# MiniMax-AI/VTP

Hardware: AMD Instinct MI355X
Metric: images/sec/node VTP-B f16d64 256x256 train step (higher is better)
Workload: dtype bf16

## Files before the change

### vtp_amd/csrc/gemm.hip

```cpp
#include "common.h"
#include "gemm_common.h"
#include <cstdlib>

namespace vtp {


template <int BM, int BN, int WAVES_M, int WAVES_N, int STAGES, int EPI, bool TRANS, bool PIPE>
__global__ __launch_bounds__(64 * WAVES_M* WAVES_N) void gemm_nt_kernel(const GemmArgs p_in) {
  constexpr int BK = 64;
  GemmArgs p = p_in;
  if constexpr (!TRANS) {
    if (p.m_rows) p.M = min(p.M, __builtin_amdgcn_readfirstlane(*p.m_rows));
  }
  constexpr int NW = WAVES_M * WAVES_N;
  constexpr int WTM = BM / WAVES_M, WTN = BN / WAVES_N;
  constexpr int TM = WTM / 32, TN = WTN / 32;
  constexpr int A_BYTES = BM * BK * 2, B_BYTES = BN * BK * 2, STAGE_BYTES = A_BYTES + B_BYTES;
  constexpr int PA = BM / 8 / NW, PB = BN / 8 / NW;
  constexpr int P = PA + PB;
  static_assert(PA >= 1 && PB >= 1 && TM >= 1 && TN >= 1, "bad tile config");
  static_assert(STAGES == 2 || STAGES == 3, "2 or 3 stages");
  extern __shared__ __attribute__((aligned(16))) char smem[];

  const int tid = threadIdx.x;
  const int lane = tid & 63;
  const int wave = __builtin_amdgcn_readfirstlane(tid >> 6);
  const int wm = wave % WAVES_M, wn = wave / WAVES_M;
  const int hi = lane >> 5;

  const int tiles_m = (p.M + BM - 1) / BM;
  const int tiles_n = (p.N + BN - 1) / BN;
  const int ntiles = tiles_m * tiles_n;
  const int G = gridDim.x;
  const int n_my = (ntiles - (int)blockIdx.x + G - 1) / G;
  auto tile_origin = [&](int i, int& m0, int& n0) {
    int wg = blockIdx.x + i * G;
    if (p.xcd_swizzle & 1) wg = xcd_chunk_start(wg, ntiles) + (wg >> 3);
    n0 = (wg % tiles_n) * BN;
    m0 = (wg / tiles_n) * BM;
  };
  const int kbeg = blockIdx.z * p.k_split;
  const int kend = min(p.K, kbeg + p.k_split);
  const int nk = (kend - kbeg + BK - 1) / BK;

  const int prow = lane >> 3;
  const int slot = lane & 7;
  const char* a_src[PA];
  const char* b_src[PB];
  int a_kc[PA], b_kc[PB];
  const char* zsrc = (const char*)g_zero_block;
  auto set_src = [&](int m0, int n0) {
    if constexpr (!TRANS) {
  #pragma unroll
      for (int i = 0; i < PA; ++i) {
        const int row = (wave * PA + i) * 8 + prow;
        const int c = slot ^ ((row >> 1) & 7);
        int m = min(m0 + row, p.M - 1);
        m = remap_row(m, p.a_grp, p.a_pre);
        a_src[i] = (const char*)(p.A + (size_t)m * p.lda + kbeg + c * 8);
        a_kc[i] = c * 8;
      }
  #pragma unroll
      for (int i = 0; i < PB; ++i) {
        const int row = (wave * PB + i) * 8 + prow;
        const int c = slot ^ ((row >> 1) & 7);
        const int n = min(n0 + row, p.N - 1);
        b_src[i] = (const char*)(p.B + (size_t)n * p.ldb + kbeg + c * 8);
        b_kc[i] = c * 8;
      }
    } else {
  #pragma unroll
      for (int i = 0; i < PA; ++i) {
        const int byte = (wave * PA + i) * 1024 + lane * 16;
        const int r = byte / (BM * 2);
        const int sp = (byte % (BM * 2)) >> 4;
        const int col = m0 + ((sp ^ (4 * (r & 3))) << 3);
        a_kc[i] = r;
        a_src[i] = col < p.M ? (const char*)(p.A + col) : nullptr;
      }
  #pragma unroll
      for (int i = 0; i < PB; ++i) {
        const int byte = (wave * PB + i) * 1024 + lane * 16;
        const int r = byte / (BN * 2);
        const int sp = (byte % (BN * 2)) >> 4;
        const int col = n0 + ((sp ^ (4 * (r & 3))) << 3);
        b_kc[i] = r;
        b_src[i] = col < p.N ? (const char*)(p.B + col) : nullptr;
      }
    }
  };

  auto stage_part = [&](int buf, int kt, int q) {
    char* abase = smem + buf * STAGE_BYTES;
    char* bbase = abase + A_BYTES;
    const int krem = kend - kbeg - kt * BK;
#pragma unroll
    for (int i = 0; i < PA; ++i) {
      if (q >= 0 && (i & 3) != q) continue;
      const char* s;
      if constexpr (!TRANS) {
        if constexpr (EPI == EPI_CONV_RELU || EPI == EPI_CONV_MASK) {
          long off = (long)kt * (BK * 2);
          if (p.conv_cin) {
            const int k0 = kt * BK, tap = k0 / p.conv_cin;
            const int ky = tap / 3, kx = tap - 3 * ky;
            off = ((long)((ky - 1) * p.conv_w2 + (kx - 1)) * p.lda + (k0 - tap * p.conv_cin)) * 2;
          }
          s = (a_kc[i] < krem) ? a_src[i] + off : zsrc;
        } else {
          s = (a_kc[i] < krem) ? a_src[i] + (size_t)kt * (BK * 2) : zsrc;
        }
      } else {
        const int t = kbeg + kt * BK + a_kc[i];
        s = (a_kc[i] < krem && a_src[i]) ? a_src[i] + (size_t)remap_row(t, p.a_grp, p.a_pre) * p.lda * 2 : zsrc;
      }
      __builtin_amdgcn_global_load_lds((const __attribute__((address_space(1))) void*)s,
                                       (__attribute__((address_space(3))) void*)(abase + (wave * PA + i) * 1024),
                                       16, 0, 0);
    }
#pragma unroll
    for (int i = 0; i < PB; ++i) {
      if (q >= 0 && ((i + PA) & 3) != q) continue;
      const char* s;
      if constexpr (!TRANS) {
        s = (b_kc[i] < krem) ? b_src[i] + (size_t)kt * (BK * 2) : zsrc;
      } else {
        const int t = kbeg + kt * BK + b_kc[i];
        s = (b_kc[i] < krem && b_src[i]) ? b_src[i] + (size_t)remap_row(t, p.b_grp, p.b_pre) * p.ldb * 2 : zsrc;
      }
      __builtin_amdgcn_global_load_lds((const __attribute__((address_space(1))) void*)s,
                                       (__attribute__((address_space(3))) void*)(bbase + (wave * PB + i) * 1024),
                                       16, 0, 0);
    }
  };
  auto stage = [&](int buf, int kt) { stage_part(buf, kt, -1); };

  f32x16 acc[TN][TM];
#pragma unroll
  for (int i = 0; i < TN; ++i)
#pragma unroll
    for (int j = 0; j < TM; ++j)
#pragma unroll
      for (int r = 0; r < 16; ++r) acc[i][j][r] = 0.f;

  const int sw = (lane >> 1) & 7;
  const int rowoff = (lane & 31) * 128;

  int s_i = 0, s_kt = 0;
  {
    int m0s, n0s;
    tile_origin(0, m0s, n0s);
    set_src(m0s, n0s);
  }
  auto advance = [&]() {
    if (++s_kt == nk) {
      s_kt = 0;
      if (++s_i < n_my) {
        int m0s, n0s;
        tile_origin(s_i, m0s, n0s);
        set_src(m0s, n0s);
      }
    }
  };
#pragma unroll
  for (int s = 0; s < STAGES - 1; ++s)
    if (s_i < n_my) {
      stage(s, s_kt);
      advance();
    }

  int buf = 0;
  int landed = 0;
  for (int ti = 0; ti < n_my; ++ti) {
  int m0, n0;
  tile_origin(ti, m0, n0);
  for (int kt = 0; kt < nk; ++kt) {
    if (landed > 0) {
      --landed;
    } else {
      const int rem = (n_my - 1 - ti) * nk + (nk - 1 - kt);
      const int later = min(STAGES - 2, rem);
      if (later >= 2) wait_vmcnt<2 * P>();
      else if (later == 1) wait_vmcnt<P>();
      else wait_vmcnt<0>();
    }
    __builtin_amdgcn_s_barrier();
    asm volatile("" ::: "memory");
    const bool prefetch = s_i < n_my;
    int nb = buf + STAGES - 1;
    if (nb >= STAGES) nb -= STAGES;
    if (!PIPE && prefetch) {
      stage(nb, s_kt);
      advance();
    }
    const char* abase = smem + buf * STAGE_BYTES;
    const char* bbase = abase + A_BYTES;

    auto load_frags = [&](int ks, bf16x8* wf, bf16x8* xf) {
      if constexpr (!TRANS) {
        const int coff = ((2 * ks + hi) ^ sw) << 4;
#pragma unroll
        for (int i = 0; i < TN; ++i)
          wf[i] = *(const bf16x8*)(bbase + (wn * WTN + i * 32) * 128 + rowoff + coff);
#pragma unroll
        for (int j = 0; j < TM; ++j)
          xf[j] = *(const bf16x8*)(abase + (wm * WTM + j * 32) * 128 + rowoff + coff);
      } else {
        const int li = lane & 15, lg = (lane >> 4) & 1;
        const int rq = li >> 2;
        const int cin = lg * 16 + (li & 3) * 4;
#pragma unroll
        for (int i = 0; i < TN; ++i) {
          const int col = wn * WTN + i * 32 + cin;
          const int soff = (((col >> 3) ^ (4 * rq)) << 4) + ((col & 7) << 1);
          const char* b0 = bbase + (ks * 16 + hi * 8 + rq) * (BN * 2) + soff;
          bf16x4 lo = __builtin_amdgcn_ds_read_tr16_b64_v4bf16((__attribute__((address_space(3))) bf16x4*)b0);
          bf16x4 hi4 = __builtin_amdgcn_ds_read_tr16_b64_v4bf16((__attribute__((address_space(3))) bf16x4*)(b0 + 4 * (BN * 2)));
          wf[i] = __builtin_shufflevector(lo, hi4, 0, 1, 2, 3, 4, 5, 6, 7);
        }
#pragma unroll
        for (int j = 0; j < TM; ++j) {
          const int col = wm * WTM + j * 32 + cin;
          const int soff = (((col >> 3) ^ (4 * rq)) << 4) + ((col & 7) << 1);
          const char* a0 = abase + (ks * 16 + hi * 8 + rq) * (BM * 2) + soff;
          bf16x4 lo = __builtin_amdgcn_ds_read_tr16_b64_v4bf16((__attribute__((address_space(3))) bf16x4*)a0);
          bf16x4 hi4 = __builtin_amdgcn_ds_read_tr16_b64_v4bf16((__attribute__((address_space(3))) bf16x4*)(a0 + 4 * (BM * 2)));
          xf[j] = __builtin_shufflevector(lo, hi4, 0, 1, 2, 3, 4, 5, 6, 7);
        }
      }
    };

    if constexpr (PIPE) {
      bf16x8 wf[2][TN], xf[2][TM];
      load_frags(0, wf[0], xf[0]);
#pragma unroll
      for (int ks = 0; ks < 4; ++ks) {
        if (ks < 3) load_frags(ks + 1, wf[(ks + 1) & 1], xf[(ks + 1) & 1]);
        if (prefetch) stage_part(nb, s_kt, ks);
#pragma unroll
        for (int i = 0; i < TN; ++i)
#pragma unroll
          for (int j = 0; j < TM; ++j)
            acc[i][j] = __builtin_amdgcn_mfma_f32_32x32x16_bf16(wf[ks & 1][i], xf[ks & 1][j], acc[i][j], 0, 0, 0);
      }
      if (prefetch) advance();
    } else {
#pragma unroll
      for (int ks = 0; ks < 4; ++ks) {
        bf16x8 wf[TN], xf[TM];
        load_frags(ks, wf, xf);
#pragma unroll
        for (int i = 0; i < TN; ++i)
#pragma unroll
          for (int j = 0; j < TM; ++j)
            acc[i][j] = __builtin_amdgcn_mfma_f32_32x32x16_bf16(wf[i], xf[j], acc[i][j], 0, 0, 0);
      }
    }
    if (++buf == STAGES) buf = 0;
  }
  if (ti + 1 < n_my) {
    wait_vmcnt<0>();
    landed = min(STAGES - 1, (n_my - 1 - ti) * nk);
  }

  {
    constexpr int REGION = STAGE_BYTES / NW;
    char* reg = nullptr;
    if (gemm_epilogue_uses_lds<EPI, TRANS, WTN, REGION>(p)) {
      const int lb = (buf == 0 ? STAGES : buf) - 1;
      __builtin_amdgcn_s_barrier();
      asm volatile("" ::: "memory");
      reg = smem + lb * STAGE_BYTES + wave * REGION;
    }
    gemm_epilogue<EPI, TRANS, WTM, WTN, REGION>(p, acc, reg, m0, n0, wm, wn, lane);
  }
#pragma unroll
  for (int i = 0; i < TN; ++i)
#pragma unroll
    for (int j = 0; j < TM; ++j)
#pragma unroll
      for (int r = 0; r < 16; ++r) acc[i][j][r] = 0.f;
  }
}

template <int BM, int BN, int WAVES_M, int WAVES_N, int STAGES, int EPI, bool TRANS, bool PIPE = false>
static int launch_cfg(const GemmArgs& a, int splits, hipStream_t s) {
  constexpr int LDS = STAGES * (BM + BN) * 64 * 2;
  static bool attr_set = false;
  auto kern = gemm_nt_kernel<BM, BN, WAVES_M, WAVES_N, STAGES, EPI, TRANS, PIPE>;
  if (!attr_set) {
    hipFuncSetAttribute((const void*)kern, hipFuncAttributeMaxDynamicSharedMemorySize, LDS);
    attr_set = true;
  }
  static int slots = 0;
  if (!slots) {
    int occ = 1, dev = 0;
    hipDeviceProp_t prop;
    (void)hipGetDevice(&dev);
    (void)hipGetDeviceProperties(&prop, dev);
    (void)hipOccupancyMaxActiveBlocksPerMultiprocessor(&occ, (const void*)kern, 64 * WAVES_M * WAVES_N, LDS);
    slots = prop.multiProcessorCount * (occ < 1 ? 1 : occ);
    slots -= slots % 8;
  }
  const int ntiles = cdiv(a.M, BM) * cdiv(a.N, BN);
  dim3 grid(splits == 1 && ntiles > slots ? slots : ntiles, 1, splits);
  hipLaunchKernelGGL(kern, grid, dim3(64 * WAVES_M * WAVES_N), LDS, s, a);
  return check_launch(TRANS ? "gemm_tn" : "gemm_nt");
}

static int g_force_cfg = -1;
static int g_xcd_swizzle = 3;
static int swz_flags() { return g_xcd_swizzle; }


int launch_gemm8p_nt(const GemmArgs& a, int epi, int splits, hipStream_t s);
int launch_gemm8p_tn(const GemmArgs& a, int epi, int splits, hipStream_t s);
bool gemm8p_fits(const GemmArgs& a, bool trans);
bool gemm8p_combine_ready(hipStream_t s);
int launch_gemm8h_nt(const GemmArgs& a, int epi, hipStream_t s);
int launch_gemm4w_nt(const GemmArgs& a, int epi, hipStream_t s);

template <int EPI, bool TRANS>
static int launch_gemm(const GemmArgs& a, int splits, int cfg, hipStream_t s) {
  if (cfg == 10) {
    if constexpr (!TRANS && (EPI == EPI_BF16 || EPI == EPI_F32 || EPI == EPI_SWIGLU || EPI == EPI_GELU)) {
      if (splits == 1 && a.N % 256 == 0 && a.K % 128 == 0 && a.a_grp == 0 && a.conv_cin == 0 && !a.timing &&
          gemm8p_fits(a, false))
        return launch_gemm4w_nt(a, EPI, s);
    }
    cfg = TRANS ? 5 : 8;
  }
  if (cfg == 9) {
    if constexpr (!TRANS && (EPI == EPI_BF16 || EPI == EPI_F32 || EPI == EPI_SWIGLU || EPI == EPI_GELU)) {
      if (splits == 1 && a.N % 256 == 0 && gemm8p_fits(a, false)) return launch_gemm8h_nt(a, EPI, s);
    }
    cfg = TRANS ? 5 : 8;
  }
  if (cfg == 8) {
    if constexpr (TRANS) {
      if (a.a_grp == 0 && a.b_grp == 0 && gemm8p_fits(a, true)) return launch_gemm8p_tn(a, EPI, splits, s);
      cfg = 5;
    } else if constexpr (EPI != EPI_CONV_RELU && EPI != EPI_CONV_MASK) {
      if (gemm8p_fits(a, false)) return launch_gemm8p_nt(a, EPI, splits, s);
      cfg = 5;
    }
  }
  if constexpr (TRANS) {
    return launch_cfg<128, 128, 4, 2, 2, EPI, true>(a, splits, s);
  } else {
    switch (cfg) {
      case 3: return launch_cfg<256, 128, 4, 2, 3, EPI, false>(a, splits, s);
      case 4:
        if constexpr (EPI == EPI_BF16) return launch_cfg<256, 128, 4, 2, 2, EPI, false>(a, splits, s);
        else return launch_cfg<256, 256, 4, 2, 2, EPI, false>(a, splits, s);
      case 5: return launch_cfg<128, 128, 4, 2, 2, EPI, false>(a, splits, s);
      case 7: return launch_cfg<128, 64, 4, 1, 3, EPI, false>(a, splits, s);
      case 21: return launch_cfg<128, 128, 4, 2, 2, EPI, false, true>(a, splits, s);
      default: return launch_cfg<128, 128, 2, 2, 2, EPI, false>(a, splits, s);
    }
  }
}

static bool use_8p_nt(int M, int N, int K, int epilogue) {
  if (N < 256 || K < 256) return false;
  const int tiles = cdiv(M, 256) * cdiv(N, 256);
  if (K < 512) return epilogue == VTP_EPI_BF16 && tiles >= 1024;
  switch (epilogue) {
    case VTP_EPI_F32: return tiles >= 128;
    case VTP_EPI_SWIGLU: return tiles >= 96;
    case VTP_EPI_BF16:
    case VTP_EPI_GELU: return tiles >= (K < 1024 ? 192 : 96);
    default: return false;
  }
}

static bool use_8h_nt(const GemmArgs& a, int epilogue) {
  if (a.N % 256 != 0 || a.N < 256 || a.K < 512) return false;
  const int t256 = cdiv(a.M, 256) * (a.N / 256), t8h = cdiv(a.M, 128) * (a.N / 256);
  if (epilogue == VTP_EPI_BF16) {
    if (a.swiglu_pre) return t256 > 256;
    if (a.rope_pos) return t256 >= 192 && t256 <= 768;
    return t256 <= 128 && t8h >= 192 && a.K <= 2304;
  }
  if (epilogue == VTP_EPI_SWIGLU) return t256 > 768 && t256 <= 1280;
  return false;
}

static bool use_8p_tn(int M, int N, int K, int splits, const GemmArgs& a) {
  if (a.a_grp || a.b_grp) return false;
  const int wgs = cdiv(M, 256) * cdiv(N, 256) * splits;
  return wgs >= 160 && wgs <= 256 && K / splits >= 1024;
}

static int combine_splits(int M, int N, int K) {
  if (N < 256 || M < 1024 || K < 4096) return 1;
  const int tiles = cdiv(M, 256) * cdiv(N, 256);
  return (tiles >= 48 && tiles <= 128) ? 2 : 1;
}

static int pick_cfg(int M, int N, int K, int epilogue, int splits) {
  if (g_force_cfg >= 0) return g_force_cfg;
  if (M < 128 || N < 128) return 0;
  if (splits > 1) return 3;
  if (use_8p_nt(M, N, K, epilogue)) return 8;
  if (cdiv(M, 256) * cdiv(N, 256) >= 384 && (N >= 2304 || K >= (epilogue == VTP_EPI_F32 ? 4096 : 2048))) return 4;
  if ((epilogue == VTP_EPI_BF16 || epilogue == VTP_EPI_F32) && K >= 512 && cdiv(M, 128) * cdiv(N, 128) < 400) return 7;
  if (K >= 4096) return 21;
  if (epilogue == VTP_EPI_SWIGLU) return 0;
  return 5;
}

static bool use_4w_nt(const GemmArgs& a, int epilogue) {
  if (epilogue != VTP_EPI_BF16 || a.rope_pos || a.swiglu_pre || a.a_grp || a.conv_cin || a.timing) return false;
  if (a.N % 256 != 0 || a.K % 128 != 0 || a.K < 2048) return false;
  return cdiv(a.M, 256) * (a.N / 256) >= 192;
}

static int pick_cfg_nt(const GemmArgs& a, int epilogue, int splits) {
  const int cfg = pick_cfg(a.M, a.N, a.K, epilogue, splits);
  static const bool use_4w = [] { const char* e = getenv("VTP_GEMM4W"); return !(e && e[0] == '0'); }();
  if (use_4w && g_force_cfg < 0 && splits == 1 && use_4w_nt(a, epilogue) && gemm8p_fits(a, false)) return 10;
  static const bool use_8h = [] { const char* e = getenv("VTP_GEMM8H"); return !(e && e[0] == '0'); }();
  if (use_8h && g_force_cfg < 0 && splits == 1 && a.a_grp == 0 && use_8h_nt(a, epilogue) && gemm8p_fits(a, false)) return 9;
  return cfg;
}

}

using namespace vtp;

template <int EPI>
static int launch_conv(const GemmArgs& a, hipStream_t s) {
  if (a.N <= 64) return launch_cfg<256, 64, 4, 2, 2, EPI, false>(a, 1, s);
  if (a.N <= 128) return launch_cfg<256, 128, 4, 2, 2, EPI, false>(a, 1, s);
  return launch_cfg<256, 256, 4, 2, 2, EPI, false>(a, 1, s);
}

extern "C" int vtp_conv3x3(const void* x, const void* w, const float* bias, void* y, const void* relu_mask, int NB, int H,
                           int W, int Cin, int Cout, int taps, int mode, void* stream) {
  VTP_REQUIRE(x && w && y, "vtp_conv3x3: null operand");
  VTP_REQUIRE(NB > 0 && H > 0 && W > 0, "vtp_conv3x3: bad shape");
  VTP_REQUIRE(taps == 9 || taps == 1, "vtp_conv3x3: taps must be 9 (3x3) or 1 (pre-unfolded rows)");
  VTP_REQUIRE(Cin % 8 == 0 && Cout % 4 == 0 && (taps == 1 || Cin % 64 == 0),
              "vtp_conv3x3: Cin must be a multiple of 64 (8 for pre-unfolded rows), Cout of 4");
  VTP_REQUIRE(mode == 0 ? bias != nullptr : true, "vtp_conv3x3: forward mode needs a bias");
  GemmArgs a{};
  a.A = (const bf16*)x; a.B = (const bf16*)w; a.C = y; a.C2 = (void*)relu_mask; a.bias = bias;
  a.M = NB * (H + 2) * (W + 2); a.N = Cout; a.K = taps * Cin;
  a.lda = Cin; a.ldb = taps * Cin; a.ldc = Cout; a.ldc2 = Cout; a.alpha = 1.f;
  a.k_split = (a.K + 63) / 64 * 64;
  a.xcd_swizzle = swz_flags();
  a.conv_cin = taps == 9 ? Cin : 0; a.conv_w2 = W + 2; a.conv_h2 = H + 2; a.conv_p = (H + 2) * (W + 2);
  hipStream_t s = (hipStream_t)stream;
  return mode == 0 ? launch_conv<EPI_CONV_RELU>(a, s) : launch_conv<EPI_CONV_MASK>(a, s);
}

extern "C" int vtp_gemm_splits(int K, int splits) {
  if (splits < 1) splits = 1;
  const int ks = ((K + splits - 1) / splits + 63) / 64 * 64;
  return (K + ks - 1) / ks;
}

extern "C" int vtp_gemm_tn_splits(int M, int N, int K) {
  const int t256 = cdiv(M, 256) * cdiv(N, 256);
  int s8 = 256 / t256;
  if (s8 > K / 1024) s8 = K / 1024;
  if (g_force_cfg < 0 && s8 >= 1) {
    const int eff = vtp_gemm_splits(K, s8);
    if (t256 * eff >= 160 && t256 * eff <= 256 && K / eff >= 1024) return eff;
  }
  const int t128 = cdiv(M, 128) * cdiv(N, 128);
  int s = 512 / t128;
  if (s > K / 512) s = K / 512;
  if (s > 16) s = 16;
  if (s < 1) s = 1;
  return vtp_gemm_splits(K, s);
}

extern "C" int vtp_set_gemm_tuning(int force_cfg, int xcd_swizzle) {
  bool known = false;
  for (int id : {-1, 0, 3, 4, 5, 7, 8, 9, 10, 21}) known |= force_cfg == id;
  VTP_REQUIRE(known, "vtp_set_gemm_tuning: force_cfg %d names no kernel configuration (-1, 0, 3, 4, 5, 7, 8, 9, 10, 21)", force_cfg);
  g_force_cfg = force_cfg;
  g_xcd_swizzle = xcd_swizzle;
  return VTP_OK;
}

extern "C" int vtp_gemm_nt_config(int M, int N, int K, int epilogue) {
  if (M <= 0 || N <= 0 || K <= 0) return -1;
  GemmArgs a{};
  a.M = M; a.N = N; a.K = K; a.lda = K; a.ldb = K;
  int cfg = pick_cfg_nt(a, epilogue, 1);
  int cs = 1;
  if (g_force_cfg < 0 && epilogue <= VTP_EPI_GELU && gemm8p_fits(a, false)) cs = combine_splits(M, N, K);
  if (cs > 1) cfg = 8;
  return cfg | (cs > 1 ? cs << 8 : 0);
}

static int gemm_nt_impl(const void* A, int lda, const void* B, int ldb, void* C, int ldc, void* C2, int ldc2,
                        const float* bias, const float* gamma, const float* resid, int M, int N, int K, int epilogue,
                        int a_grp, int a_pre, int c_grp, int c_pre, int splits, float alpha, const int* m_rows, void* stream) {
  VTP_REQUIRE(A && B && C, "vtp_gemm_nt: null operand");
  VTP_REQUIRE(M > 0 && N > 0 && K > 0, "vtp_gemm_nt: bad shape M=%d N=%d K=%d", M, N, K);
  const int act_quick = epilogue == VTP_EPI_QUICK_GELU;
  if (act_quick) epilogue = VTP_EPI_GELU;
  VTP_REQUIRE(K % 8 == 0 && lda % 8 == 0 && ldb % 8 == 0, "vtp_gemm_nt: K, lda, ldb must be multiples of 8 (16-B rows)");
  VTP_REQUIRE(N % 4 == 0 && ldc % 4 == 0, "vtp_gemm_nt: N and ldc must be multiples of 4");
  VTP_REQUIRE(((uintptr_t)A % 16 == 0) && ((uintptr_t)B % 16 == 0) && ((uintptr_t)C % 16 == 0), "vtp_gemm_nt: operands must be 16-B aligned");
  VTP_REQUIRE(splits >= 1, "vtp_gemm_nt: splits must be >= 1");
  VTP_REQUIRE(splits == 1 || epilogue == VTP_EPI_F32_ATOMIC || epilogue == VTP_EPI_F32_SLAB,
              "vtp_gemm_nt: split-K needs the atomic or slab epilogue");
  VTP_REQUIRE(epilogue != VTP_EPI_F32_SLAB || (ldc2 > 0), "vtp_gemm_nt: slab epilogue needs ldc2 = slab stride / 4 (in float4 units)");
  GemmArgs a{};
  a.A = (const bf16*)A; a.B = (const bf16*)B; a.C = C; a.C2 = C2; a.bias = bias; a.gamma = gamma; a.resid = resid;
  a.M = M; a.N = N; a.K = K; a.lda = lda; a.ldb = ldb; a.ldc = ldc; a.ldc2 = ldc2;
  a.a_grp = a_grp; a.a_pre = a_pre; a.c_grp = c_grp; a.c_pre = c_pre; a.alpha = alpha;
  a.b_grp = 0; a.b_pre = 0;
  a.act_quick = act_quick;
  a.xcd_swizzle = swz_flags();
  int ks = ((K + splits - 1) / splits + 63) / 64 * 64;
  a.k_split = ks;
  splits = (K + ks - 1) / ks;
  hipStream_t s = (hipStream_t)stream;
  int cfg = pick_cfg_nt(a, epilogue, splits);
  int cs = 1;
  if (splits == 1 && g_force_cfg < 0 && epilogue <= VTP_EPI_GELU && gemm8p_fits(a, false)) cs = combine_splits(M, N, K);
  if (cs > 1 && !gemm8p_combine_ready(s)) cs = 1;
  if (cs > 1) {
    a.k_split = ((K + cs - 1) / cs + 63) / 64 * 64;
    cs = (K + a.k_split - 1) / a.k_split;
    cfg = 8;
  }
  if (m_rows) {
    VTP_REQUIRE(splits == 1 && epilogue <= VTP_EPI_GELU && a_grp == 0 && c_grp == 0,
                "vtp_gemm_nt_limit: a row limit needs one K slice, a plain / fp32 / SwiGLU / GELU epilogue and no row remaps");
    VTP_REQUIRE(g_force_cfg < 8, "vtp_gemm_nt_limit: the forced configuration %d takes no row limit (ring configurations only)", g_force_cfg);
    if (cs > 1) {
      cs = 1;
      a.k_split = ks;
    }
    if (cfg >= 8) {
      cfg = pick_cfg(M, N, K, epilogue, 1);
      if (cfg >= 8) cfg = K >= 4096 ? 21 : 5;
    }
    a.m_rows = m_rows;
  }
  switch (epilogue) {
    case VTP_EPI_BF16: return launch_gemm<EPI_BF16, false>(a, cs, cfg, s);
    case VTP_EPI_F32: return launch_gemm<EPI_F32, false>(a, cs, cfg, s);
    case VTP_EPI_SWIGLU:
      VTP_REQUIRE(N % 16 == 0 && bias, "vtp_gemm_nt: SwiGLU epilogue needs interleaved N %% 16 == 0 and a bias");
      return launch_gemm<EPI_SWIGLU, false>(a, cs, cfg, s);
    case VTP_EPI_GELU: return launch_gemm<EPI_GELU, false>(a, cs, cfg, s);
    case VTP_EPI_F32_ATOMIC: return launch_gemm<EPI_F32_ATOMIC, false>(a, splits, cfg, s);
    case VTP_EPI_F32_SLAB: return launch_gemm<EPI_F32_SLAB, false>(a, splits, cfg, s);
    default: VTP_REQUIRE(false, "vtp_gemm_nt: unknown epilogue %d", epilogue);
  }
  return VTP_OK;
}

extern "C" int vtp_gemm_nt(const void* A, int lda, const void* B, int ldb, void* C, int ldc, void* C2, int ldc2,
                           const float* bias, const float* gamma, const float* resid, int M, int N, int K, int epilogue,
                           int a_grp, int a_pre, int c_grp, int c_pre, int splits, float alpha, void* stream) {
  return gemm_nt_impl(A, lda, B, ldb, C, ldc, C2, ldc2, bias, gamma, resid, M, N, K, epilogue, a_grp, a_pre, c_grp, c_pre, splits,
                      alpha, nullptr, stream);
}

extern "C" int vtp_gemm_nt_limit(const void* A, int lda, const void* B, int ldb, void* C, int ldc, void* C2, int ldc2,
                                const float* bias, const float* gamma, const float* resid, int M, int N, int K, int epilogue,
                                float alpha, const int* m_rows, void* stream) {
  VTP_REQUIRE(m_rows, "vtp_gemm_nt_limit: null row count");
  return gemm_nt_impl(A, lda, B, ldb, C, ldc, C2, ldc2, bias, gamma, resid, M, N, K, epilogue, 0, 0, 0, 0, 1, alpha, m_rows, stream);
}

extern "C" int vtp_gemm_dgrad_swiglu(const void* A, int lda, const void* WT, int ldb, const void* x12, int ldx, void* dx12, int ldc,
                                     int M, int H, int K, void* stream) {
  VTP_REQUIRE(A && WT && x12 && dx12, "vtp_gemm_dgrad_swiglu: null operand");
  VTP_REQUIRE(M > 0 && H > 0 && K > 0 && H % 8 == 0 && K % 8 == 0 && lda % 8 == 0 && ldb % 8 == 0 && ldx % 8 == 0 && ldc % 8 == 0 &&
              ldx >= 2 * H && ldc >= 2 * H, "vtp_gemm_dgrad_swiglu: H, K and the leading dimensions must be multiples of 8, ldx / ldc >= 2 H");
  VTP_REQUIRE(((uintptr_t)A % 16 == 0) && ((uintptr_t)WT % 16 == 0) && ((uintptr_t)x12 % 16 == 0) && ((uintptr_t)dx12 % 16 == 0),
              "vtp_gemm_dgrad_swiglu: operands must be 16-B aligned");
  GemmArgs a{};
  a.A = (const bf16*)A; a.B = (const bf16*)WT; a.C = dx12;
  a.M = M; a.N = H; a.K = K; a.lda = lda; a.ldb = ldb; a.ldc = ldc; a.alpha = 1.f;
  a.xcd_swizzle = swz_flags() | 2;
  a.k_split = (K + 63) / 64 * 64;
  a.swiglu_pre = (const bf16*)x12; a.swiglu_ld = ldx;
  return launch_gemm<EPI_BF16, false>(a, 1, pick_cfg_nt(a, VTP_EPI_BF16, 1), (hipStream_t)stream);
}

namespace vtp {
int launch_gemm8p_nt_fp8(const GemmArgs& a, int epi, hipStream_t s);
}
extern "C" int vtp_gemm_nt_fp8(const void* A8, int lda, const void* B8, int ldb, void* C, int ldc, void* C2, int ldc2,
                               const float* bias, const float* resid, int M, int N, int K, int epilogue, float alpha,
                               const int* rope_pos, const void* rope_sin, const void* rope_cos, int rope_cols, void* stream) {
  VTP_REQUIRE(A8 && B8 && C, "vtp_gemm_nt_fp8: null operand");
  VTP_REQUIRE(!rope_pos || (epilogue == VTP_EPI_BF16 && rope_sin && rope_cos && rope_cols % 128 == 0 && rope_cols <= N && N % 8 == 0 &&
                            ldc % 8 == 0), "vtp_gemm_nt_fp8: fused RoPE needs the bf16 epilogue, both tables and rope_cols %% 128 == 0");
  VTP_REQUIRE(M > 0 && N > 0 && K > 0, "vtp_gemm_nt_fp8: bad shape M=%d N=%d K=%d", M, N, K);
  VTP_REQUIRE(K % 16 == 0 && lda % 16 == 0 && ldb % 16 == 0, "vtp_gemm_nt_fp8: K, lda, ldb must be multiples of 16 (16-B rows)");
  VTP_REQUIRE(N % 4 == 0 && ldc % 4 == 0, "vtp_gemm_nt_fp8: N and ldc must be multiples of 4");
  VTP_REQUIRE(((uintptr_t)A8 % 16 == 0) && ((uintptr_t)B8 % 16 == 0) && ((uintptr_t)C % 16 == 0), "vtp_gemm_nt_fp8: operands must be 16-B aligned");
  VTP_REQUIRE(epilogue == VTP_EPI_BF16 || epilogue == VTP_EPI_F32 || epilogue == VTP_EPI_SWIGLU, "vtp_gemm_nt_fp8: forward epilogues only");
  VTP_REQUIRE(epilogue != VTP_EPI_SWIGLU || (N % 16 == 0 && bias), "vtp_gemm_nt_fp8: SwiGLU epilogue needs interleaved N %% 16 == 0 and a bias");
  GemmArgs a{};
  a.A = (const bf16*)A8; a.B = (const bf16*)B8; a.C = C; a.C2 = C2; a.bias = bias; a.resid = resid;
  a.M = M; a.N = N; a.K = K / 2; a.lda = lda / 2; a.ldb = ldb / 2; a.ldc = ldc; a.ldc2 = ldc2;
  a.alpha = alpha;
  a.xcd_swizzle = swz_flags();
  a.k_split = (a.K + 63) / 64 * 64;
  if (rope_pos) {
    a.xcd_swizzle |= 2;
    a.rope_pos = rope_pos; a.rope_sin = (const bf16*)rope_sin; a.rope_cos = (const bf16*)rope_cos; a.rope_cols = rope_cols;
  }
  return launch_gemm8p_nt_fp8(a, epilogue, (hipStream_t)stream);
}

extern "C" int vtp_gemm_qkv_rope(const void* A, int lda, const void* W, int ldb, const float* bias, void* C, int ldc, int M, int N,
                                 int K, const int* rope_pos, const void* rope_sin, const void* rope_cos, int rope_cols,
                                 void* stream) {
  VTP_REQUIRE(A && W && C && rope_pos && rope_sin && rope_cos, "vtp_gemm_qkv_rope: null operand");
  VTP_REQUIRE(M > 0 && N > 0 && K > 0, "vtp_gemm_qkv_rope: bad shape M=%d N=%d K=%d", M, N, K);
  VTP_REQUIRE(K % 8 == 0 && lda % 8 == 0 && ldb % 8 == 0 && N % 8 == 0 && ldc % 8 == 0, "vtp_gemm_qkv_rope: K, N, lda, ldb, ldc must be multiples of 8");
  VTP_REQUIRE(rope_cols % 128 == 0 && rope_cols <= N, "vtp_gemm_qkv_rope: rope_cols must be a multiple of 128 (head_dim 64, two heads per 128-column wave tile)");
  VTP_REQUIRE(((uintptr_t)A % 16 == 0) && ((uintptr_t)W % 16 == 0) && ((uintptr_t)C % 16 == 0) && ((uintptr_t)rope_sin % 16 == 0) &&
              ((uintptr_t)rope_cos % 16 == 0), "vtp_gemm_qkv_rope: operands must be 16-B aligned");
  GemmArgs a{};
  a.A = (const bf16*)A; a.B = (const bf16*)W; a.C = C; a.bias = bias;
  a.M = M; a.N = N; a.K = K; a.lda = lda; a.ldb = ldb; a.ldc = ldc; a.alpha = 1.f;
  a.xcd_swizzle = swz_flags() | 2;
  a.k_split = (K + 63) / 64 * 64;
  a.rope_pos = rope_pos; a.rope_sin = (const bf16*)rope_sin; a.rope_cos = (const bf16*)rope_cos; a.rope_cols = rope_cols;
  return launch_gemm<EPI_BF16, false>(a, 1, pick_cfg_nt(a, VTP_EPI_BF16, 1), (hipStream_t)stream);
}

extern "C" int vtp_colsum_bf16(const void* in, int ld, float* out, int colsum_swiglu_h, int in_grp, int in_pre, int R, int C,
                               void* stream);

extern "C" int vtp_gemm_tn(const void* A, int lda, const void* B, int ldb, void* C, int ldc, int ldc2, const float* resid,
                           int M, int N, int K, int epilogue, int a_grp, int a_pre, int b_grp, int b_pre, int c_grp, int c_pre,
                           int splits, float* a_colsum, void* stream) {
  VTP_REQUIRE(A && B && C, "vtp_gemm_tn: null operand");
  VTP_REQUIRE(M > 0 && N > 0 && K > 0, "vtp_gemm_tn: bad shape M=%d N=%d K=%d", M, N, K);
  VTP_REQUIRE(M % 8 == 0 && N % 8 == 0 && lda % 8 == 0 && ldb % 8 == 0 && ldc % 4 == 0, "vtp_gemm_tn: M, N, lda, ldb must be multiples of 8");
  VTP_REQUIRE(((uintptr_t)A % 16 == 0) && ((uintptr_t)B % 16 == 0) && ((uintptr_t)C % 16 == 0), "vtp_gemm_tn: operands must be 16-B aligned");
  VTP_REQUIRE(epilogue == VTP_EPI_F32 || epilogue == VTP_EPI_F32_SLAB || epilogue == VTP_EPI_F32_ATOMIC,
              "vtp_gemm_tn: epilogue must be F32 (accumulate via resid), F32_SLAB or F32_ATOMIC");
  VTP_REQUIRE(splits >= 1 && (splits == 1 || epilogue != VTP_EPI_F32), "vtp_gemm_tn: split-K needs the slab or the atomic epilogue");
  VTP_REQUIRE(epilogue != VTP_EPI_F32_SLAB || ldc2 > 0, "vtp_gemm_tn: slab epilogue needs ldc2 = slab stride / 4");
  GemmArgs a{};
  a.A = (const bf16*)A; a.B = (const bf16*)B; a.C = C; a.C2 = nullptr; a.bias = nullptr; a.gamma = nullptr; a.resid = resid;
  a.M = M; a.N = N; a.K = K; a.lda = lda; a.ldb = ldb; a.ldc = ldc; a.ldc2 = ldc2;
  a.a_grp = a_grp; a.a_pre = a_pre; a.b_grp = b_grp; a.b_pre = b_pre; a.c_grp = c_grp; a.c_pre = c_pre; a.alpha = 1.f;
  a.xcd_swizzle = swz_flags();
  int ks = ((K + splits - 1) / splits + 63) / 64 * 64;
  a.k_split = ks;
  splits = (K + ks - 1) / ks;
  int cfg = g_force_cfg >= 0 ? g_force_cfg : (use_8p_tn(M, N, K, splits, a) ? 8 : 5);
  if (cfg != 8) cfg = 5;
  hipStream_t s = (hipStream_t)stream;
  if (a_colsum) {
    VTP_REQUIRE(c_grp <= 0, "vtp_gemm_tn: a_colsum supports the identity and the SwiGLU (c_grp = -1) row maps only");
    if (cfg == 8 && a_grp == 0 && b_grp == 0 && gemm8p_fits(a, true)) {
      a.colsum = a_colsum;
    } else {
      const int rc = vtp_colsum_bf16(A, lda, a_colsum, c_grp < 0 ? c_pre : 0, a_grp, a_pre, K, M, stream);
      if (rc != VTP_OK) return rc;
    }
  }
  if (epilogue == VTP_EPI_F32) return launch_gemm<EPI_F32, true>(a, 1, cfg, s);
  if (epilogue == VTP_EPI_F32_ATOMIC) return launch_gemm<EPI_F32_ATOMIC, true>(a, splits, cfg, s);
  return launch_gemm<EPI_F32_SLAB, true>(a, splits, cfg, s);
}
```

### vtp_amd/csrc/gemm4w.hip

```cpp
#include "gemm_common.h"
#include "gemm4w_ktile.inc"
#include <type_traits>
#include <utility>

namespace vtp {

namespace {
constexpr int W4_IMG = 16384;
constexpr int W4_KT = 4 * W4_IMG;
constexpr int W4_RING = 2 * W4_KT;
constexpr int W4_REGION = 8192;
constexpr int W4_LDS = W4_RING + 4 * W4_REGION;
}

__device__ __forceinline__ void w4_glds16(const char* sbase, unsigned voff, unsigned lds_dst) {
  unsigned keep;
  asm volatile("s_mov_b32 %0, m0\n\ts_mov_b32 m0, %3\n\ts_nop 0\n\tglobal_load_lds_dwordx4 %1, %2\n\ts_mov_b32 m0, %0"
               : "=&s"(keep)
               : "v"(voff), "s"(sbase), "s"(lds_dst)
               : "memory");
}
__device__ __forceinline__ void w4_mfma_drain() {
  asm volatile("s_nop 15\n\ts_nop 15\n\ts_nop 7" ::: "memory");
}

struct W4Cursor {
  unsigned pea, poa, peb, pob, cc;
};
struct W4Stage {
  const char *mata, *matb;
  unsigned stepa, stepb, kadva, kadvb, da[2], db[2];
};
__device__ __forceinline__ void w4_tile_kloop(f32x16 (&acc)[4][4], bf16x8 (&fl)[8], bf16x8 (&fp)[16], const unsigned (&adX)[2][4],
                                              const unsigned (&adY)[2][4], W4Cursor& cur, const W4Stage& st, unsigned vmaxa, unsigned vmaxb,
                                              unsigned tadva, unsigned tadvb, unsigned nk) {
  bf16x8 fh[8], fq[16];
  unsigned t0, t1, sm, sadva, sadvb, cnt = nk >> 1;
  asm volatile(W4_TILE_ASM
               : W4_TILE_OUTS, [pea] "+v"(cur.pea), [poa] "+v"(cur.poa), [peb] "+v"(cur.peb), [pob] "+v"(cur.pob), [vt0] "=&v"(t0),
                 [vt1] "=&v"(t1), [cc] "+s"(cur.cc), [cnt] "+s"(cnt), [sm] "=&s"(sm), [sadva] "=&s"(sadva), [sadvb] "=&s"(sadvb)
               : W4_TILE_ADDRS, [vmaxa] "v"(vmaxa), [vmaxb] "v"(vmaxb), [mata] "s"(st.mata), [matb] "s"(st.matb), [stepa] "s"(st.stepa),
                 [stepb] "s"(st.stepb), [kadva] "s"(st.kadva), [kadvb] "s"(st.kadvb), [tadva] "s"(tadva), [tadvb] "s"(tadvb), [nkr] "s"(nk),
                 [da0] "s"(st.da[0]), [da1] "s"(st.da[1]), [db0] "s"(st.db[0]), [db1] "s"(st.db[1])
               : "memory", "scc");
}

template <int... Is, class F>
__device__ __forceinline__ void w4_for(std::integer_sequence<int, Is...>, F&& f) {
  (f(std::integral_constant<int, Is>{}), ...);
}

template <int EPI, int XMODE, bool DYN = false>
__global__ __launch_bounds__(256, 1) void gemm4w_kernel(const GemmArgs p) {
  extern __shared__ __attribute__((aligned(16))) char smem[];
  const int tid = threadIdx.x;
  const int lane = tid & 63;
  const int wave = __builtin_amdgcn_readfirstlane(tid >> 6);
  const int wr = wave >> 1, wc = wave & 1;

  const int tiles_m = (p.M + 255) >> 8;
  const int tiles_n = (p.N + 255) >> 8;
  const int ntiles = tiles_m * tiles_n;
  const int G = gridDim.x, bx = blockIdx.x;
  const int n_my = DYN ? 0x10000 : (ntiles - bx + G - 1) / G;
  int d_cur = -1, d_next = -1, d_idx = 0;
  bool d_more = DYN;
  auto pos_origin = [&](int wg, int& m0, int& n0) {
    n0 = (wg % tiles_n) << 8;
    m0 = (wg / tiles_n) << 8;
  };
  auto tile_origin = [&](int i, int& m0, int& n0) {
    if constexpr (DYN) {
      pos_origin((i > d_idx && d_next >= 0) ? d_next : d_cur, m0, n0);
      return;
    }
    int wg = bx + i * G;
    if (p.xcd_swizzle & 1) wg = xcd_chunk_start(wg, ntiles) + (wg >> 3);
    pos_origin(wg, m0, n0);
  };
  const TileQueue tq = DYN ? TileQueue(p.tq, (int*)(smem + W4_RING), ntiles, bx) : TileQueue();
  if constexpr (DYN) {
    const int j = tq.first(tid);
    if (j >= tq.n) {
      tq.leave(tid, G);
      return;
    }
    d_cur = tq.start + j;
    d_more = j + 1 < tq.n;
    d_next = d_more ? d_cur + 1 : -1;
  }
  const int nk = p.K >> 6;

  const int prow = lane >> 3;
  const int share = (wave >> 1) * 128 + (wave & 1) * 64;
  const unsigned step8a = (unsigned)(8 * p.lda * 2), step8b = (unsigned)(8 * p.ldb * 2);
  const unsigned offa_e = (unsigned)((prow * p.lda + (((lane & 7) ^ (prow >> 1)) << 3)) * 2);
  const unsigned offa_o = (unsigned)((prow * p.lda + (((lane & 7) ^ (prow >> 1) ^ 4) << 3)) * 2) + step8a;
  const unsigned offb_e = (unsigned)((prow * p.ldb + (((lane & 7) ^ (prow >> 1)) << 3)) * 2);
  const unsigned offb_o = (unsigned)((prow * p.ldb + (((lane & 7) ^ (prow >> 1) ^ 4) << 3)) * 2) + step8b;
  const unsigned vmaxa = (unsigned)(((size_t)(p.M - 1) * p.lda + p.K - 8) * 2), vmaxb = (unsigned)(((size_t)(p.N - 1) * p.ldb + p.K - 8) * 2);
  auto tile_off = [&](int i, unsigned& oa, unsigned& ob) {
    int m0s, n0s;
    tile_origin(DYN ? i : (i < n_my ? i : n_my - 1), m0s, n0s);
    oa = (unsigned)(m0s + share) * (unsigned)(p.lda * 2);
    ob = (unsigned)(n0s + share) * (unsigned)(p.ldb * 2);
  };
  W4Stage st;
  st.mata = (const char*)p.A;
  st.matb = (const char*)p.B;
  st.stepa = 2 * step8a;
  st.stepb = 2 * step8b;
  st.kadva = 128u - 8u * step8a;
  st.kadvb = 128u - 8u * step8b;
#pragma unroll
  for (int sl = 0; sl < 2; ++sl) {
    st.da[sl] = (unsigned)(size_t)smem + sl * W4_KT + (wave >> 1) * W4_IMG + (wave & 1) * 8192;
    st.db[sl] = st.da[sl] + 2 * W4_IMG;
  }
  int s_i = 0, s_c = 0;
  auto issue_ktile = [&](int slot) {
    unsigned oa, ob;
    tile_off(s_i, oa, ob);
    w4_for(std::make_integer_sequence<int, 8>{}, [&](auto it) {
      constexpr int I = decltype(it)::value;
      w4_glds16(st.mata, min(oa + s_c * 128 + (I & ~1) * step8a + ((I & 1) ? offa_o : offa_e), vmaxa), st.da[slot] + I * 1024);
      w4_glds16(st.matb, min(ob + s_c * 128 + (I & ~1) * step8b + ((I & 1) ? offb_o : offb_e), vmaxb), st.db[slot] + I * 1024);
    });
    if (++s_c == nk) {
      s_c = 0;
      ++s_i;
    }
  };

  bf16x8 fl[8], fp[16];
  f32x16 acc[4][4];
  auto zero_acc = [&]() {
#pragma unroll
    for (int i = 0; i < 4; ++i)
#pragma unroll
      for (int j = 0; j < 4; ++j)
#pragma unroll
        for (int r = 0; r < 16; ++r) acc[i][j][r] = 0.f;
  };
  zero_acc();

  issue_ktile(0);
  issue_ktile(1);
  W4Cursor cur;
  {
    unsigned oa, ob;
    tile_off(s_i, oa, ob);
    cur.pea = oa + s_c * 128 + offa_e;
    cur.poa = oa + s_c * 128 + offa_o;
    cur.peb = ob + s_c * 128 + offb_e;
    cur.pob = ob + s_c * 128 + offb_o;
  }
  asm volatile("s_waitcnt vmcnt(0)" ::: "memory");
  __builtin_amdgcn_s_barrier();
  __builtin_amdgcn_sched_barrier(0);
  for (int ti = 0; ti < n_my; ++ti) {
    int m0, n0;
    tile_origin(ti, m0, n0);
    int ln = lane;
    asm volatile("" : "+v"(ln));
    const int sw = (ln >> 1) & 7, rowoff = (ln & 31) * 128, hi2 = ln >> 5;
    unsigned adX[2][4], adY[2][4];
#pragma unroll
    for (int sl = 0; sl < 2; ++sl)
#pragma unroll
      for (int ks = 0; ks < 4; ++ks) {
        const unsigned lo = rowoff + (((2 * ks + hi2) ^ sw) << 4);
        adX[sl][ks] = (unsigned)(size_t)smem + sl * W4_KT + wr * W4_IMG + lo;
        adY[sl][ks] = (unsigned)(size_t)smem + sl * W4_KT + (2 + wc) * W4_IMG + lo;
      }
#pragma unroll
    for (int ks = 0; ks < 4; ++ks) {
      const int lo = rowoff + (((2 * ks + hi2) ^ sw) << 4);
#pragma unroll
      for (int b = 0; b < 2; ++b) fl[ks * 2 + b] = *(const bf16x8*)(smem + wr * W4_IMG + b * 4096 + lo);
#pragma unroll
      for (int i = 0; i < 4; ++i) fp[ks * 4 + i] = *(const bf16x8*)(smem + (2 + wc) * W4_IMG + i * 4096 + lo);
    }
    cur.cc = (unsigned)(nk - s_c);
    unsigned oa0, ob0, oa1, ob1;
    tile_off(s_i, oa0, ob0);
    tile_off(s_i + 1, oa1, ob1);
    const unsigned back = (unsigned)(nk - 1) * 128u;
    w4_tile_kloop(acc, fl, fp, adX, adY, cur, st, vmaxa, vmaxb, oa1 - oa0 - back - 8u * step8a, ob1 - ob0 - back - 8u * step8b, (unsigned)nk);
    if (s_i < n_my) ++s_i;
    w4_mfma_drain();
    const int d_t = DYN ? tq.draw(d_more, tid) : 0;
    char* reg = gemm_epilogue_uses_lds<EPI, false, 64, 4096>(p) ? smem + W4_RING + wave * W4_REGION : nullptr;
    char* reg2 = (EPI == EPI_SWIGLU && reg) ? reg + 4096 : nullptr;
    if constexpr (EPI == EPI_BF16 && XMODE != 2) {
      char* reg8 = gemm_epilogue_uses_lds<EPI, false, 128, W4_REGION>(p) ? smem + W4_RING + wave * W4_REGION : nullptr;
      gemm_epilogue<EPI, false, 128, 128, W4_REGION, XMODE>(p, acc, reg8, m0, n0, wr, wc, lane, 0, nullptr);
    } else {
      gemm_epilogue<EPI, false, 128, 64, 4096, XMODE>(p, *(f32x16(*)[2][4]) & acc[0], reg, m0, n0, wr, wc * 2, lane, 0, reg2);
      gemm_epilogue<EPI, false, 128, 64, 4096, XMODE>(p, *(f32x16(*)[2][4]) & acc[2], reg, m0, n0, wr, wc * 2 + 1, lane, 0, reg2);
    }
    zero_acc();
    if constexpr (DYN) {
      tq.post(d_more, tid, d_t);
      __syncthreads();
      const int nn = d_more ? tq.take() : -1;
      __syncthreads();
      d_cur = d_next;
      d_next = nn;
      d_more = nn >= 0;
      ++d_idx;
      if (d_cur < 0) break;
    }
  }
  asm volatile("s_waitcnt vmcnt(0)" ::: "memory");
  if constexpr (DYN) tq.leave(tid, G);
}

template <int EPI, int XMODE = 0>
static int launch4w(const GemmArgs& a, hipStream_t s) {
  const int ntiles = cdiv(a.M, 256) * cdiv(a.N, 256);
  return launch_persistent<gemm4w_kernel<EPI, XMODE>, gemm4w_kernel<EPI, XMODE, true>>(a, ntiles, 1, 256, W4_LDS, 4, s, "gemm4w_nt");
}

int launch_gemm4w_nt(const GemmArgs& a, int epi, hipStream_t s) {
  switch (epi) {
    case EPI_BF16:
      if (a.rope_pos) return launch4w<EPI_BF16, 1>(a, s);
      if (a.swiglu_pre) return launch4w<EPI_BF16, 2>(a, s);
      return launch4w<EPI_BF16, 0>(a, s);
    case EPI_F32: return launch4w<EPI_F32>(a, s);
    case EPI_SWIGLU: return launch4w<EPI_SWIGLU>(a, s);
    case EPI_GELU: return launch4w<EPI_GELU>(a, s);
    default: set_error("gemm4w: unsupported epilogue %d", epi); return VTP_ERR_ARG;
  }
}

}
```

Baseline: 753.7.

## Add 16x16x32 MFMA variant of 4-wave persistent GEMM for bf16 epilogue

Adds a new configuration (11) of the 4-wave persistent NT GEMM whose inner k-loop uses v_mfma_f32_16x16x32_bf16 on an 8x8 grid of 16x16 accumulator blocks instead of 32x32 MFMAs. It also adds a matching LDS fragment addressing scheme and a dedicated bf16 epilogue with bias. It becomes the default for plain bf16-epilogue GEMMs that would have used config 10, with an environment variable to opt out. The aim is higher MFMA throughput or better issue interleaving on MI355X. The cost is more MFMA instructions and different register pressure, plus a new hand-scheduled assembly loop that must stay correct.

```diff
diff --git a/vtp_amd/csrc/gemm.hip b/vtp_amd/csrc/gemm.hip
--- a/vtp_amd/csrc/gemm.hip
+++ b/vtp_amd/csrc/gemm.hip
@@ -319,9 +319,26 @@
 bool gemm8p_combine_ready(hipStream_t s);
 int launch_gemm8h_nt(const GemmArgs& a, int epi, hipStream_t s);
 int launch_gemm4w_nt(const GemmArgs& a, int epi, hipStream_t s);
+int launch_gemm4w16_nt(const GemmArgs& a, hipStream_t s);
+
+static bool use_mfma16_4w() {
+  static const bool on = [] { const char* e = getenv("VTP_GEMM4W_MFMA"); return !(e && e[0] == '3'); }();
+  return on;
+}
 
 template <int EPI, bool TRANS>
 static int launch_gemm(const GemmArgs& a, int splits, int cfg, hipStream_t s) {
+  if constexpr (!TRANS && EPI == EPI_BF16) {
+    if (cfg == 10 && g_force_cfg < 0 && !a.rope_pos && !a.swiglu_pre && use_mfma16_4w()) cfg = 11;
+  }
+  if (cfg == 11) {
+    if constexpr (!TRANS && EPI == EPI_BF16) {
+      if (splits == 1 && a.N % 256 == 0 && a.K % 128 == 0 && a.a_grp == 0 && a.conv_cin == 0 && !a.timing && !a.rope_pos &&
+          !a.swiglu_pre && gemm8p_fits(a, false))
+        return launch_gemm4w16_nt(a, s);
+    }
+    cfg = 5;
+  }
   if (cfg == 10) {
     if constexpr (!TRANS && (EPI == EPI_BF16 || EPI == EPI_F32 || EPI == EPI_SWIGLU || EPI == EPI_GELU)) {
       if (splits == 1 && a.N % 256 == 0 && a.K % 128 == 0 && a.a_grp == 0 && a.conv_cin == 0 && !a.timing &&
@@ -479,8 +496,8 @@
 
 extern "C" int vtp_set_gemm_tuning(int force_cfg, int xcd_swizzle) {
   bool known = false;
-  for (int id : {-1, 0, 3, 4, 5, 7, 8, 9, 10, 21}) known |= force_cfg == id;
-  VTP_REQUIRE(known, "vtp_set_gemm_tuning: force_cfg %d names no kernel configuration (-1, 0, 3, 4, 5, 7, 8, 9, 10, 21)", force_cfg);
+  for (int id : {-1, 0, 3, 4, 5, 7, 8, 9, 10, 11, 21}) known |= force_cfg == id;
+  VTP_REQUIRE(known, "vtp_set_gemm_tuning: force_cfg %d names no kernel configuration (-1, 0, 3, 4, 5, 7, 8, 9, 10, 11, 21)", force_cfg);
   g_force_cfg = force_cfg;
   g_xcd_swizzle = xcd_swizzle;
   return VTP_OK;
diff --git a/vtp_amd/csrc/gemm4w.hip b/vtp_amd/csrc/gemm4w.hip
--- a/vtp_amd/csrc/gemm4w.hip
+++ b/vtp_amd/csrc/gemm4w.hip
@@ -1,5 +1,6 @@
 #include "gemm_common.h"
 #include "gemm4w_ktile.inc"
+#include "gemm4w16_ktile.inc"
 #include <type_traits>
 #include <utility>
 
@@ -45,13 +46,79 @@
                : "memory", "scc");
 }
 
+__device__ __forceinline__ void w16_tile_kloop(f32x4 (&acc)[8][8], bf16x8 (&fl)[8], bf16x8 (&fp)[16], const unsigned (&adX)[2][2],
+                                               const unsigned (&adY)[2][2], W4Cursor& cur, const W4Stage& st, unsigned vmaxa, unsigned vmaxb,
+                                               unsigned tadva, unsigned tadvb, unsigned nk) {
+  bf16x8 fh[8], fq[16];
+  unsigned t0, t1, sm, sadva, sadvb, cnt = nk >> 1;
+  asm volatile(W16_TILE_ASM
+               : W16_TILE_OUTS, [pea] "+v"(cur.pea), [poa] "+v"(cur.poa), [peb] "+v"(cur.peb), [pob] "+v"(cur.pob), [vt0] "=&v"(t0),
+                 [vt1] "=&v"(t1), [cc] "+s"(cur.cc), [cnt] "+s"(cnt), [sm] "=&s"(sm), [sadva] "=&s"(sadva), [sadvb] "=&s"(sadvb)
+               : W16_TILE_ADDRS, [vmaxa] "v"(vmaxa), [vmaxb] "v"(vmaxb), [mata] "s"(st.mata), [matb] "s"(st.matb), [stepa] "s"(st.stepa),
+                 [stepb] "s"(st.stepb), [kadva] "s"(st.kadva), [kadvb] "s"(st.kadvb), [tadva] "s"(tadva), [tadvb] "s"(tadvb), [nkr] "s"(nk),
+                 [da0] "s"(st.da[0]), [da1] "s"(st.da[1]), [db0] "s"(st.db[0]), [db1] "s"(st.db[1])
+               : "memory", "scc");
+}
+
+__device__ __forceinline__ void w16_epilogue_bf16(const GemmArgs& p, f32x4 (&acc)[8][8], char* reg, int m0, int n0, int wr, int wc, int lane_in) {
+  int lane = lane_in;
+  asm volatile("" : "+v"(lane));
+  const int r16 = lane & 15, g = lane >> 4;
+  f32x4 bias_v[8];
+#pragma unroll
+  for (int i = 0; i < 8; ++i) {
+    const int n = n0 + wc * 128 + i * 16 + 4 * g;
+    bias_v[i] = (p.bias && n < p.N) ? *(const f32x4*)(p.bias + n) : f32x4{0.f, 0.f, 0.f, 0.f};
+  }
+  if (reg) {
+    constexpr int RB = 256, CPR = 16, TPB = 32 * CPR / 64;
+#pragma unroll
+    for (int jb = 0; jb < 4; ++jb) {
+#pragma unroll
+      for (int jj = 0; jj < 2; ++jj)
+#pragma unroll
+        for (int i = 0; i < 8; ++i) {
+          const int rr = jj * 16 + r16;
+          f32x4 v = acc[i][2 * jb + jj] * p.alpha;
+          v += bias_v[i];
+          *(bf16x4*)(reg + rr * RB + (((2 * i + (g >> 1)) ^ (rr & (CPR - 1))) << 4) + (g & 1) * 8) = __builtin_convertvector(v, bf16x4);
+        }
+#pragma unroll
+      for (int t = 0; t < TPB; ++t) {
+        const int idx = t * 64 + lane, rr = idx / CPR, c = idx % CPR;
+        const bf16x8 val = *(const bf16x8*)(reg + rr * RB + ((c ^ (rr & (CPR - 1))) << 4));
+        const int m = m0 + wr * 128 + jb * 32 + rr, n = n0 + wc * 128 + c * 8;
+        if (m < p.M && n < p.N) *(bf16x8*)((bf16*)p.C + (size_t)remap_row(m, p.c_grp, p.c_pre) * p.ldc + n) = val;
+      }
+    }
+    return;
+  }
+#pragma unroll
+  for (int j = 0; j < 8; ++j) {
+    const int m = m0 + wr * 128 + j * 16 + r16;
+    if (m >= p.M) continue;
+    bf16* crow = (bf16*)p.C + (size_t)remap_row(m, p.c_grp, p.c_pre) * p.ldc;
+#pragma unroll
+    for (int i = 0; i < 8; ++i) {
+      const int n = n0 + wc * 128 + i * 16 + 4 * g;
+      if (n >= p.N) continue;
+      f32x4 v = acc[i][j] * p.alpha;
+      v += bias_v[i];
+      *(bf16x4*)(crow + n) = __builtin_convertvector(v, bf16x4);
+    }
+  }
+}
+
 template <int... Is, class F>
 __device__ __forceinline__ void w4_for(std::integer_sequence<int, Is...>, F&& f) {
   (f(std::integral_constant<int, Is>{}), ...);
 }
 
+constexpr int W4_MF16 = 16;
 template <int EPI, int XMODE, bool DYN = false>
 __global__ __launch_bounds__(256, 1) void gemm4w_kernel(const GemmArgs p) {
+  constexpr bool MF16 = XMODE == W4_MF16;
+  static_assert(!MF16 || EPI == EPI_BF16, "configuration 11 has the plain bf16 epilogue only");
   extern __shared__ __attribute__((aligned(16))) char smem[];
   const int tid = threadIdx.x;
   const int lane = tid & 63;
@@ -133,14 +200,15 @@
   };
 
   bf16x8 fl[8], fp[16];
-  f32x16 acc[4][4];
+  constexpr int NB = MF16 ? 8 : 4, NR = MF16 ? 4 : 16, NKS = MF16 ? 2 : 4;
+  std::conditional_t<MF16, f32x4, f32x16> acc[NB][NB];
   auto zero_acc = [&]() {
 #pragma unroll
-    for (int i = 0; i < 4; ++i)
-#pragma unroll
-      for (int j = 0; j < 4; ++j)
-#pragma unroll
-        for (int r = 0; r < 16; ++r) acc[i][j][r] = 0.f;
+    for (int i = 0; i < NB; ++i)
+#pragma unroll
+      for (int j = 0; j < NB; ++j)
+#pragma unroll
+        for (int r = 0; r < NR; ++r) acc[i][j][r] = 0.f;
   };
   zero_acc();
 
@@ -163,36 +231,43 @@
     tile_origin(ti, m0, n0);
     int ln = lane;
     asm volatile("" : "+v"(ln));
-    const int sw = (ln >> 1) & 7, rowoff = (ln & 31) * 128, hi2 = ln >> 5;
-    unsigned adX[2][4], adY[2][4];
+    const int sw = (ln >> 1) & 7, rowoff = (MF16 ? ln & 15 : ln & 31) * 128, hi2 = MF16 ? ln >> 4 : ln >> 5;
+    constexpr int CPK = 8 / NKS, BLK = W4_IMG / NB;
+    unsigned adX[2][NKS], adY[2][NKS];
 #pragma unroll
     for (int sl = 0; sl < 2; ++sl)
 #pragma unroll
-      for (int ks = 0; ks < 4; ++ks) {
-        const unsigned lo = rowoff + (((2 * ks + hi2) ^ sw) << 4);
+      for (int ks = 0; ks < NKS; ++ks) {
+        const unsigned lo = rowoff + (((CPK * ks + hi2) ^ sw) << 4);
         adX[sl][ks] = (unsigned)(size_t)smem + sl * W4_KT + wr * W4_IMG + lo;
         adY[sl][ks] = (unsigned)(size_t)smem + sl * W4_KT + (2 + wc) * W4_IMG + lo;
       }
 #pragma unroll
-    for (int ks = 0; ks < 4; ++ks) {
-      const int lo = rowoff + (((2 * ks + hi2) ^ sw) << 4);
-#pragma unroll
-      for (int b = 0; b < 2; ++b) fl[ks * 2 + b] = *(const bf16x8*)(smem + wr * W4_IMG + b * 4096 + lo);
-#pragma unroll
-      for (int i = 0; i < 4; ++i) fp[ks * 4 + i] = *(const bf16x8*)(smem + (2 + wc) * W4_IMG + i * 4096 + lo);
+    for (int ks = 0; ks < NKS; ++ks) {
+      const int lo = rowoff + (((CPK * ks + hi2) ^ sw) << 4);
+#pragma unroll
+      for (int b = 0; b < NB / 2; ++b) fl[ks * (NB / 2) + b] = *(const bf16x8*)(smem + wr * W4_IMG + b * BLK + lo);
+#pragma unroll
+      for (int i = 0; i < NB; ++i) fp[ks * NB + i] = *(const bf16x8*)(smem + (2 + wc) * W4_IMG + i * BLK + lo);
     }
     cur.cc = (unsigned)(nk - s_c);
     unsigned oa0, ob0, oa1, ob1;
     tile_off(s_i, oa0, ob0);
     tile_off(s_i + 1, oa1, ob1);
     const unsigned back = (unsigned)(nk - 1) * 128u;
-    w4_tile_kloop(acc, fl, fp, adX, adY, cur, st, vmaxa, vmaxb, oa1 - oa0 - back - 8u * step8a, ob1 - ob0 - back - 8u * step8b, (unsigned)nk);
+    if constexpr (MF16)
+      w16_tile_kloop(acc, fl, fp, adX, adY, cur, st, vmaxa, vmaxb, oa1 - oa0 - back - 8u * step8a, ob1 - ob0 - back - 8u * step8b, (unsigned)nk);
+    else
+      w4_tile_kloop(acc, fl, fp, adX, adY, cur, st, vmaxa, vmaxb, oa1 - oa0 - back - 8u * step8a, ob1 - ob0 - back - 8u * step8b, (unsigned)nk);
     if (s_i < n_my) ++s_i;
     w4_mfma_drain();
     const int d_t = DYN ? tq.draw(d_more, tid) : 0;
     char* reg = gemm_epilogue_uses_lds<EPI, false, 64, 4096>(p) ? smem + W4_RING + wave * W4_REGION : nullptr;
     char* reg2 = (EPI == EPI_SWIGLU && reg) ? reg + 4096 : nullptr;
-    if constexpr (EPI == EPI_BF16 && XMODE != 2) {
+    if constexpr (MF16) {
+      w16_epilogue_bf16(p, acc, gemm_epilogue_uses_lds<EPI, false, 128, W4_REGION>(p) ? smem + W4_RING + wave * W4_REGION : nullptr, m0, n0,
+                        wr, wc, lane);
+    } else if constexpr (EPI == EPI_BF16 && XMODE != 2) {
       char* reg8 = gemm_epilogue_uses_lds<EPI, false, 128, W4_REGION>(p) ? smem + W4_RING + wave * W4_REGION : nullptr;
       gemm_epilogue<EPI, false, 128, 128, W4_REGION, XMODE>(p, acc, reg8, m0, n0, wr, wc, lane, 0, nullptr);
     } else {
@@ -222,6 +297,11 @@
   return launch_persistent<gemm4w_kernel<EPI, XMODE>, gemm4w_kernel<EPI, XMODE, true>>(a, ntiles, 1, 256, W4_LDS, 4, s, "gemm4w_nt");
 }
 
+int launch_gemm4w16_nt(const GemmArgs& a, hipStream_t s) {
+  const int ntiles = cdiv(a.M, 256) * cdiv(a.N, 256);
+  return launch_persistent<gemm4w_kernel<EPI_BF16, W4_MF16>, gemm4w_kernel<EPI_BF16, W4_MF16, true>>(a, ntiles, 1, 256, W4_LDS, 4, s, "gemm4w16_nt");
+}
+
 int launch_gemm4w_nt(const GemmArgs& a, int epi, hipStream_t s) {
   switch (epi) {
     case EPI_BF16:
diff --git a/vtp_amd/csrc/gemm4w16_ktile.inc b/vtp_amd/csrc/gemm4w16_ktile.inc
--- /dev/null
+++ b/vtp_amd/csrc/gemm4w16_ktile.inc
@@ -0,0 +1,485 @@
+#define W16_TILE_ASM \
+  "s_mov_b32 %[sm], m0\n\t" \
+  "1:\n\t" \
+  "s_waitcnt lgkmcnt(0)\n\t" \
+  "s_barrier\n\t" \
+  "s_mov_b32 m0, %[db0]\n\t" \
+  "v_min_u32 %[vt0], %[peb], %[vmaxb]\n\t" \
+  "v_mfma_f32_16x16x32_bf16 %[c00], %[p0], %[l0], %[c00]\n\t" \
+  "ds_read_b128 %[h0], %[x00] offset:8192\n\t" \
+  "v_mfma_f32_16x16x32_bf16 %[c10], %[p1], %[l0], %[c10]\n\t" \
+  "v_mfma_f32_16x16x32_bf16 %[c20], %[p2], %[l0], %[c20]\n\t" \
+  "global_load_lds_dwordx4 %[vt0], %[matb]\n\t" \
+  "v_add_u32 %[peb], %[stepb], %[peb]\n\t" \
+  "v_mfma_f32_16x16x32_bf16 %[c30], %[p3], %[l0], %[c30]\n\t" \
+  "v_mfma_f32_16x16x32_bf16 %[c40], %[p4], %[l0], %[c40]\n\t" \
+  "ds_read_b128 %[h1], %[x00] offset:10240\n\t" \
+  "v_mfma_f32_16x16x32_bf16 %[c50], %[p5], %[l0], %[c50]\n\t" \
+  "v_mfma_f32_16x16x32_bf16 %[c60], %[p6], %[l0], %[c60]\n\t" \
+  "v_mfma_f32_16x16x32_bf16 %[c70], %[p7], %[l0], %[c70]\n\t" \
+  "s_add_u32 m0, m0, 0x400\n\t" \
+  "v_min_u32 %[vt1], %[pob], %[vmaxb]\n\t" \
+  "v_mfma_f32_16x16x32_bf16 %[c01], %[p0], %[l1], %[c01]\n\t" \
+  "ds_read_b128 %[h2], %[x00] offset:12288\n\t" \
+  "v_mfma_f32_16x16x32_bf16 %[c11], %[p1], %[l1], %[c11]\n\t" \
+  "v_mfma_f32_16x16x32_bf16 %[c21], %[p2], %[l1], %[c21]\n\t" \
+  "global_load_lds_dwordx4 %[vt1], %[matb]\n\t" \
+  "v_add_u32 %[pob], %[stepb], %[pob]\n\t" \
+  "v_mfma_f32_16x16x32_bf16 %[c31], %[p3], %[l1], %[c31]\n\t" \
+  "v_mfma_f32_16x16x32_bf16 %[c41], %[p4], %[l1], %[c41]\n\t" \
+  "ds_read_b128 %[h3], %[x00] offset:14336\n\t" \
+  "v_mfma_f32_16x16x32_bf16 %[c51], %[p5], %[l1], %[c51]\n\t" \
+  "v_mfma_f32_16x16x32_bf16 %[c61], %[p6], %[l1], %[c61]\n\t" \
+  "v_mfma_f32_16x16x32_bf16 %[c71], %[p7], %[l1], %[c71]\n\t" \
+  "s_add_u32 m0, m0, 0x400\n\t" \
+  "v_min_u32 %[vt0], %[peb], %[vmaxb]\n\t" \
+  "v_mfma_f32_16x16x32_bf16 %[c02], %[p0], %[l2], %[c02]\n\t" \
+  "ds_read_b128 %[h4], %[x01] offset:8192\n\t" \
+  "v_mfma_f32_16x16x32_bf16 %[c12], %[p1], %[l2], %[c12]\n\t" \
+  "v_mfma_f32_16x16x32_bf16 %[c22], %[p2], %[l2], %[c22]\n\t" \
+  "global_load_lds_dwordx4 %[vt0], %[matb]\n\t" \
+  "v_add_u32 %[peb], %[stepb], %[peb]\n\t" \
+  "v_mfma_f32_16x16x32_bf16 %[c32], %[p3], %[l2], %[c32]\n\t" \
+  "v_mfma_f32_16x16x32_bf16 %[c42], %[p4], %[l2], %[c42]\n\t" \
+  "ds_read_b128 %[h5], %[x01] offset:10240\n\t" \
+  "v_mfma_f32_16x16x32_bf16 %[c52], %[p5], %[l2], %[c52]\n\t" \
+  "v_mfma_f32_16x16x32_bf16 %[c62], %[p6], %[l2], %[c62]\n\t" \
+  "v_mfma_f32_16x16x32_bf16 %[c72], %[p7], %[l2], %[c72]\n\t" \
+  "s_add_u32 m0, m0, 0x400\n\t" \
+  "v_min_u32 %[vt1], %[pob], %[vmaxb]\n\t" \
+  "v_mfma_f32_16x16x32_bf16 %[c03], %[p0], %[l3], %[c03]\n\t" \
+  "ds_read_b128 %[h6], %[x01] offset:12288\n\t" \
+  "v_mfma_f32_16x16x32_bf16 %[c13], %[p1], %[l3], %[c13]\n\t" \
+  "v_mfma_f32_16x16x32_bf16 %[c23], %[p2], %[l3], %[c23]\n\t" \
+  "global_load_lds_dwordx4 %[vt1], %[matb]\n\t" \
+  "v_add_u32 %[pob], %[stepb], %[pob]\n\t" \
+  "v_mfma_f32_16x16x32_bf16 %[c33], %[p3], %[l3], %[c33]\n\t" \
+  "v_mfma_f32_16x16x32_bf16 %[c43], %[p4], %[l3], %[c43]\n\t" \
+  "ds_read_b128 %[h7], %[x01] offset:14336\n\t" \
+  "v_mfma_f32_16x16x32_bf16 %[c53], %[p5], %[l3], %[c53]\n\t" \
+  "v_mfma_f32_16x16x32_bf16 %[c63], %[p6], %[l3], %[c63]\n\t" \
+  "v_mfma_f32_16x16x32_bf16 %[c73], %[p7], %[l3], %[c73]\n\t" \
+  "s_add_u32 m0, m0, 0x400\n\t" \
+  "v_min_u32 %[vt0], %[peb], %[vmaxb]\n\t" \
+  "v_mfma_f32_16x16x32_bf16 %[c00], %[p8], %[l4], %[c00]\n\t" \
+  "v_mfma_f32_16x16x32_bf16 %[c10], %[p9], %[l4], %[c10]\n\t" \
+  "v_mfma_f32_16x16x32_bf16 %[c20], %[p10], %[l4], %[c20]\n\t" \
+  "global_load_lds_dwordx4 %[vt0], %[matb]\n\t" \
+  "v_add_u32 %[peb], %[stepb], %[peb]\n\t" \
+  "v_mfma_f32_16x16x32_bf16 %[c30], %[p11], %[l4], %[c30]\n\t" \
+  "v_mfma_f32_16x16x32_bf16 %[c40], %[p12], %[l4], %[c40]\n\t" \
+  "v_mfma_f32_16x16x32_bf16 %[c50], %[p13], %[l4], %[c50]\n\t" \
+  "v_mfma_f32_16x16x32_bf16 %[c60], %[p14], %[l4], %[c60]\n\t" \
+  "v_mfma_f32_16x16x32_bf16 %[c70], %[p15], %[l4], %[c70]\n\t" \
+  "s_add_u32 m0, m0, 0x400\n\t" \
+  "v_min_u32 %[vt1], %[pob], %[vmaxb]\n\t" \
+  "v_mfma_f32_16x16x32_bf16 %[c01], %[p8], %[l5], %[c01]\n\t" \
+  "v_mfma_f32_16x16x32_bf16 %[c11], %[p9], %[l5], %[c11]\n\t" \
+  "v_mfma_f32_16x16x32_bf16 %[c21], %[p10], %[l5], %[c21]\n\t" \
+  "global_load_lds_dwordx4 %[vt1], %[matb]\n\t" \
+  "v_add_u32 %[pob], %[stepb], %[pob]\n\t" \
+  "v_mfma_f32_16x16x32_bf16 %[c31], %[p11], %[l5], %[c31]\n\t" \
+  "v_mfma_f32_16x16x32_bf16 %[c41], %[p12], %[l5], %[c41]\n\t" \
+  "v_mfma_f32_16x16x32_bf16 %[c51], %[p13], %[l5], %[c51]\n\t" \
+  "v_mfma_f32_16x16x32_bf16 %[c61], %[p14], %[l5], %[c61]\n\t" \
+  "v_mfma_f32_16x16x32_bf16 %[c71], %[p15], %[l5], %[c71]\n\t" \
+  "s_add_u32 m0, m0, 0x400\n\t" \
+  "v_min_u32 %[vt0], %[peb], %[vmaxb]\n\t" \
+  "v_mfma_f32_16x16x32_bf16 %[c02], %[p8], %[l6], %[c02]\n\t" \
+  "v_mfma_f32_16x16x32_bf16 %[c12], %[p9], %[l6], %[c12]\n\t" \
+  "v_mfma_f32_16x16x32_bf16 %[c22], %[p10], %[l6], %[c22]\n\t" \
+  "global_load_lds_dwordx4 %[vt0], %[matb]\n\t" \
+  "v_add_u32 %[peb], %[stepb], %[peb]\n\t" \
+  "v_mfma_f32_16x16x32_bf16 %[c32], %[p11], %[l6], %[c32]\n\t" \
+  "v_mfma_f32_16x16x32_bf16 %[c42], %[p12], %[l6], %[c42]\n\t" \
+  "v_mfma_f32_16x16x32_bf16 %[c52], %[p13], %[l6], %[c52]\n\t" \
+  "v_mfma_f32_16x16x32_bf16 %[c62], %[p14], %[l6], %[c62]\n\t" \
+  "v_mfma_f32_16x16x32_bf16 %[c72], %[p15], %[l6], %[c72]\n\t" \
+  "s_add_u32 m0, m0, 0x400\n\t" \
+  "v_min_u32 %[vt1], %[pob], %[vmaxb]\n\t" \
+  "v_mfma_f32_16x16x32_bf16 %[c03], %[p8], %[l7], %[c03]\n\t" \
+  "v_mfma_f32_16x16x32_bf16 %[c13], %[p9], %[l7], %[c13]\n\t" \
+  "v_mfma_f32_16x16x32_bf16 %[c23], %[p10], %[l7], %[c23]\n\t" \
+  "global_load_lds_dwordx4 %[vt1], %[matb]\n\t" \
+  "v_add_u32 %[pob], %[stepb], %[pob]\n\t" \
+  "v_mfma_f32_16x16x32_bf16 %[c33], %[p11], %[l7], %[c33]\n\t" \
+  "v_mfma_f32_16x16x32_bf16 %[c43], %[p12], %[l7], %[c43]\n\t" \
+  "v_mfma_f32_16x16x32_bf16 %[c53], %[p13], %[l7], %[c53]\n\t" \
+  "v_mfma_f32_16x16x32_bf16 %[c63], %[p14], %[l7], %[c63]\n\t" \
+  "v_mfma_f32_16x16x32_bf16 %[c73], %[p15], %[l7], %[c73]\n\t" \
+  "s_sub_u32 %[cc], %[cc], 1\n\t" \
+  "s_cmp_eq_u32 %[cc], 0\n\t" \
+  "s_cselect_b32 %[sadvb], %[tadvb], %[kadvb]\n\t" \
+  "s_cselect_b32 %[sadva], %[tadva], %[kadva]\n\t" \
+  "s_cselect_b32 %[cc], %[nkr], %[cc]\n\t" \
+  "v_add_u32 %[peb], %[sadvb], %[peb]\n\t" \
+  "v_add_u32 %[pob], %[sadvb], %[pob]\n\t" \
+  "s_waitcnt vmcnt(8) lgkmcnt(0)\n\t" \
+  "s_barrier\n\t" \
+  "s_mov_b32 m0, %[da0]\n\t" \
+  "v_min_u32 %[vt0], %[pea], %[vmaxa]\n\t" \
+  "v_mfma_f32_16x16x32_bf16 %[c04], %[p0], %[h0], %[c04]\n\t" \
+  "ds_read_b128 %[l0], %[x10] offset:0\n\t" \
+  "v_mfma_f32_16x16x32_bf16 %[c14], %[p1], %[h0], %[c14]\n\t" \
+  "ds_read_b128 %[l1], %[x10] offset:2048\n\t" \
+  "v_mfma_f32_16x16x32_bf16 %[c24], %[p2], %[h0], %[c24]\n\t" \
+  "global_load_lds_dwordx4 %[vt0], %[mata]\n\t" \
+  "v_add_u32 %[pea], %[stepa], %[pea]\n\t" \
+  "v_mfma_f32_16x16x32_bf16 %[c34], %[p3], %[h0], %[c34]\n\t" \
+  "v_mfma_f32_16x16x32_bf16 %[c44], %[p4], %[h0], %[c44]\n\t" \
+  "ds_read_b128 %[l2], %[x10] offset:4096\n\t" \
+  "v_mfma_f32_16x16x32_bf16 %[c54], %[p5], %[h0], %[c54]\n\t" \
+  "ds_read_b128 %[l3], %[x10] offset:6144\n\t" \
+  "v_mfma_f32_16x16x32_bf16 %[c64], %[p6], %[h0], %[c64]\n\t" \
+  "v_mfma_f32_16x16x32_bf16 %[c74], %[p7], %[h0], %[c74]\n\t" \
+  "s_add_u32 m0, m0, 0x400\n\t" \
+  "v_min_u32 %[vt1], %[poa], %[vmaxa]\n\t" \
+  "v_mfma_f32_16x16x32_bf16 %[c05], %[p0], %[h1], %[c05]\n\t" \
+  "ds_read_b128 %[q0], %[y10] offset:0\n\t" \
+  "v_mfma_f32_16x16x32_bf16 %[c15], %[p1], %[h1], %[c15]\n\t" \
+  "ds_read_b128 %[q1], %[y10] offset:2048\n\t" \
+  "v_mfma_f32_16x16x32_bf16 %[c25], %[p2], %[h1], %[c25]\n\t" \
+  "global_load_lds_dwordx4 %[vt1], %[mata]\n\t" \
+  "v_add_u32 %[poa], %[stepa], %[poa]\n\t" \
+  "v_mfma_f32_16x16x32_bf16 %[c35], %[p3], %[h1], %[c35]\n\t" \
+  "v_mfma_f32_16x16x32_bf16 %[c45], %[p4], %[h1], %[c45]\n\t" \
+  "ds_read_b128 %[q2], %[y10] offset:4096\n\t" \
+  "v_mfma_f32_16x16x32_bf16 %[c55], %[p5], %[h1], %[c55]\n\t" \
+  "ds_read_b128 %[q3], %[y10] offset:6144\n\t" \
+  "v_mfma_f32_16x16x32_bf16 %[c65], %[p6], %[h1], %[c65]\n\t" \
+  "v_mfma_f32_16x16x32_bf16 %[c75], %[p7], %[h1], %[c75]\n\t" \
+  "s_add_u32 m0, m0, 0x400\n\t" \
+  "v_min_u32 %[vt0], %[pea], %[vmaxa]\n\t" \
+  "v_mfma_f32_16x16x32_bf16 %[c06], %[p0], %[h2], %[c06]\n\t" \
+  "ds_read_b128 %[q4], %[y10] offset:8192\n\t" \
+  "v_mfma_f32_16x16x32_bf16 %[c16], %[p1], %[h2], %[c16]\n\t" \
+  "ds_read_b128 %[q5], %[y10] offset:10240\n\t" \
+  "v_mfma_f32_16x16x32_bf16 %[c26], %[p2], %[h2], %[c26]\n\t" \
+  "global_load_lds_dwordx4 %[vt0], %[mata]\n\t" \
+  "v_add_u32 %[pea], %[stepa], %[pea]\n\t" \
+  "v_mfma_f32_16x16x32_bf16 %[c36], %[p3], %[h2], %[c36]\n\t" \
+  "v_mfma_f32_16x16x32_bf16 %[c46], %[p4], %[h2], %[c46]\n\t" \
+  "ds_read_b128 %[q6], %[y10] offset:12288\n\t" \
+  "v_mfma_f32_16x16x32_bf16 %[c56], %[p5], %[h2], %[c56]\n\t" \
+  "ds_read_b128 %[q7], %[y10] offset:14336\n\t" \
+  "v_mfma_f32_16x16x32_bf16 %[c66], %[p6], %[h2], %[c66]\n\t" \
+  "v_mfma_f32_16x16x32_bf16 %[c76], %[p7], %[h2], %[c76]\n\t" \
+  "s_add_u32 m0, m0, 0x400\n\t" \
+  "v_min_u32 %[vt1], %[poa], %[vmaxa]\n\t" \
+  "v_mfma_f32_16x16x32_bf16 %[c07], %[p0], %[h3], %[c07]\n\t" \
+  "ds_read_b128 %[l4], %[x11] offset:0\n\t" \
+  "v_mfma_f32_16x16x32_bf16 %[c17], %[p1], %[h3], %[c17]\n\t" \
+  "ds_read_b128 %[l5], %[x11] offset:2048\n\t" \
+  "v_mfma_f32_16x16x32_bf16 %[c27], %[p2], %[h3], %[c27]\n\t" \
+  "global_load_lds_dwordx4 %[vt1], %[mata]\n\t" \
+  "v_add_u32 %[poa], %[stepa], %[poa]\n\t" \
+  "v_mfma_f32_16x16x32_bf16 %[c37], %[p3], %[h3], %[c37]\n\t" \
+  "v_mfma_f32_16x16x32_bf16 %[c47], %[p4], %[h3], %[c47]\n\t" \
+  "ds_read_b128 %[l6], %[x11] offset:4096\n\t" \
+  "v_mfma_f32_16x16x32_bf16 %[c57], %[p5], %[h3], %[c57]\n\t" \
+  "ds_read_b128 %[l7], %[x11] offset:6144\n\t" \
+  "v_mfma_f32_16x16x32_bf16 %[c67], %[p6], %[h3], %[c67]\n\t" \
+  "v_mfma_f32_16x16x32_bf16 %[c77], %[p7], %[h3], %[c77]\n\t" \
+  "s_add_u32 m0, m0, 0x400\n\t" \
+  "v_min_u32 %[vt0], %[pea], %[vmaxa]\n\t" \
+  "v_mfma_f32_16x16x32_bf16 %[c04], %[p8], %[h4], %[c04]\n\t" \
+  "ds_read_b128 %[q8], %[y11] offset:0\n\t" \
+  "v_mfma_f32_16x16x32_bf16 %[c14], %[p9], %[h4], %[c14]\n\t" \
+  "ds_read_b128 %[q9], %[y11] offset:2048\n\t" \
+  "v_mfma_f32_16x16x32_bf16 %[c24], %[p10], %[h4], %[c24]\n\t" \
+  "global_load_lds_dwordx4 %[vt0], %[mata]\n\t" \
+  "v_add_u32 %[pea], %[stepa], %[pea]\n\t" \
+  "v_mfma_f32_16x16x32_bf16 %[c34], %[p11], %[h4], %[c34]\n\t" \
+  "v_mfma_f32_16x16x32_bf16 %[c44], %[p12], %[h4], %[c44]\n\t" \
+  "ds_read_b128 %[q10], %[y11] offset:4096\n\t" \
+  "v_mfma_f32_16x16x32_bf16 %[c54], %[p13], %[h4], %[c54]\n\t" \
+  "ds_read_b128 %[q11], %[y11] offset:6144\n\t" \
+  "v_mfma_f32_16x16x32_bf16 %[c64], %[p14], %[h4], %[c64]\n\t" \
+  "v_mfma_f32_16x16x32_bf16 %[c74], %[p15], %[h4], %[c74]\n\t" \
+  "s_add_u32 m0, m0, 0x400\n\t" \
+  "v_min_u32 %[vt1], %[poa], %[vmaxa]\n\t" \
+  "v_mfma_f32_16x16x32_bf16 %[c05], %[p8], %[h5], %[c05]\n\t" \
+  "ds_read_b128 %[q12], %[y11] offset:8192\n\t" \
+  "v_mfma_f32_16x16x32_bf16 %[c15], %[p9], %[h5], %[c15]\n\t" \
+  "ds_read_b128 %[q13], %[y11] offset:10240\n\t" \
+  "v_mfma_f32_16x16x32_bf16 %[c25], %[p10], %[h5], %[c25]\n\t" \
+  "global_load_lds_dwordx4 %[vt1], %[mata]\n\t" \
+  "v_add_u32 %[poa], %[stepa], %[poa]\n\t" \
+  "v_mfma_f32_16x16x32_bf16 %[c35], %[p11], %[h5], %[c35]\n\t" \
+  "v_mfma_f32_16x16x32_bf16 %[c45], %[p12], %[h5], %[c45]\n\t" \
+  "ds_read_b128 %[q14], %[y11] offset:12288\n\t" \
+  "v_mfma_f32_16x16x32_bf16 %[c55], %[p13], %[h5], %[c55]\n\t" \
+  "ds_read_b128 %[q15], %[y11] offset:14336\n\t" \
+  "v_mfma_f32_16x16x32_bf16 %[c65], %[p14], %[h5], %[c65]\n\t" \
+  "v_mfma_f32_16x16x32_bf16 %[c75], %[p15], %[h5], %[c75]\n\t" \
+  "s_add_u32 m0, m0, 0x400\n\t" \
+  "v_min_u32 %[vt0], %[pea], %[vmaxa]\n\t" \
+  "v_mfma_f32_16x16x32_bf16 %[c06], %[p8], %[h6], %[c06]\n\t" \
+  "v_mfma_f32_16x16x32_bf16 %[c16], %[p9], %[h6], %[c16]\n\t" \
+  "v_mfma_f32_16x16x32_bf16 %[c26], %[p10], %[h6], %[c26]\n\t" \
+  "global_load_lds_dwordx4 %[vt0], %[mata]\n\t" \
+  "v_add_u32 %[pea], %[stepa], %[pea]\n\t" \
+  "v_mfma_f32_16x16x32_bf16 %[c36], %[p11], %[h6], %[c36]\n\t" \
+  "v_mfma_f32_16x16x32_bf16 %[c46], %[p12], %[h6], %[c46]\n\t" \
+  "v_mfma_f32_16x16x32_bf16 %[c56], %[p13], %[h6], %[c56]\n\t" \
+  "v_mfma_f32_16x16x32_bf16 %[c66], %[p14], %[h6], %[c66]\n\t" \
+  "v_mfma_f32_16x16x32_bf16 %[c76], %[p15], %[h6], %[c76]\n\t" \
+  "s_add_u32 m0, m0, 0x400\n\t" \
+  "v_min_u32 %[vt1], %[poa], %[vmaxa]\n\t" \
+  "v_mfma_f32_16x16x32_bf16 %[c07], %[p8], %[h7], %[c07]\n\t" \
+  "v_mfma_f32_16x16x32_bf16 %[c17], %[p9], %[h7], %[c17]\n\t" \
+  "v_mfma_f32_16x16x32_bf16 %[c27], %[p10], %[h7], %[c27]\n\t" \
+  "global_load_lds_dwordx4 %[vt1], %[mata]\n\t" \
+  "v_add_u32 %[poa], %[stepa], %[poa]\n\t" \
+  "v_mfma_f32_16x16x32_bf16 %[c37], %[p11], %[h7], %[c37]\n\t" \
+  "v_mfma_f32_16x16x32_bf16 %[c47], %[p12], %[h7], %[c47]\n\t" \
+  "v_mfma_f32_16x16x32_bf16 %[c57], %[p13], %[h7], %[c57]\n\t" \
+  "v_mfma_f32_16x16x32_bf16 %[c67], %[p14], %[h7], %[c67]\n\t" \
+  "v_mfma_f32_16x16x32_bf16 %[c77], %[p15], %[h7], %[c77]\n\t" \
+  "v_add_u32 %[pea], %[sadva], %[pea]\n\t" \
+  "v_add_u32 %[poa], %[sadva], %[poa]\n\t" \
+  "s_waitcnt lgkmcnt(0)\n\t" \
+  "s_barrier\n\t" \
+  "s_mov_b32 m0, %[db1]\n\t" \
+  "v_min_u32 %[vt0], %[peb], %[vmaxb]\n\t" \
+  "v_mfma_f32_16x16x32_bf16 %[c00], %[q0], %[l0], %[c00]\n\t" \
+  "ds_read_b128 %[h0], %[x10] offset:8192\n\t" \
+  "v_mfma_f32_16x16x32_bf16 %[c10], %[q1], %[l0], %[c10]\n\t" \
+  "v_mfma_f32_16x16x32_bf16 %[c20], %[q2], %[l0], %[c20]\n\t" \
+  "global_load_lds_dwordx4 %[vt0], %[matb]\n\t" \
+  "v_add_u32 %[peb], %[stepb], %[peb]\n\t" \
+  "v_mfma_f32_16x16x32_bf16 %[c30], %[q3], %[l0], %[c30]\n\t" \
+  "v_mfma_f32_16x16x32_bf16 %[c40], %[q4], %[l0], %[c40]\n\t" \
+  "ds_read_b128 %[h1], %[x10] offset:10240\n\t" \
+  "v_mfma_f32_16x16x32_bf16 %[c50], %[q5], %[l0], %[c50]\n\t" \
+  "v_mfma_f32_16x16x32_bf16 %[c60], %[q6], %[l0], %[c60]\n\t" \
+  "v_mfma_f32_16x16x32_bf16 %[c70], %[q7], %[l0], %[c70]\n\t" \
+  "s_add_u32 m0, m0, 0x400\n\t" \
+  "v_min_u32 %[vt1], %[pob], %[vmaxb]\n\t" \
+  "v_mfma_f32_16x16x32_bf16 %[c01], %[q0], %[l1], %[c01]\n\t" \
+  "ds_read_b128 %[h2], %[x10] offset:12288\n\t" \
+  "v_mfma_f32_16x16x32_bf16 %[c11], %[q1], %[l1], %[c11]\n\t" \
+  "v_mfma_f32_16x16x32_bf16 %[c21], %[q2], %[l1], %[c21]\n\t" \
+  "global_load_lds_dwordx4 %[vt1], %[matb]\n\t" \
+  "v_add_u32 %[pob], %[stepb], %[pob]\n\t" \
+  "v_mfma_f32_16x16x32_bf16 %[c31], %[q3], %[l1], %[c31]\n\t" \
+  "v_mfma_f32_16x16x32_bf16 %[c41], %[q4], %[l1], %[c41]\n\t" \
+  "ds_read_b128 %[h3], %[x10] offset:14336\n\t" \
+  "v_mfma_f32_16x16x32_bf16 %[c51], %[q5], %[l1], %[c51]\n\t" \
+  "v_mfma_f32_16x16x32_bf16 %[c61], %[q6], %[l1], %[c61]\n\t" \
+  "v_mfma_f32_16x16x32_bf16 %[c71], %[q7], %[l1], %[c71]\n\t" \
+  "s_add_u32 m0, m0, 0x400\n\t" \
+  "v_min_u32 %[vt0], %[peb], %[vmaxb]\n\t" \
+  "v_mfma_f32_16x16x32_bf16 %[c02], %[q0], %[l2], %[c02]\n\t" \
+  "ds_read_b128 %[h4], %[x11] offset:8192\n\t" \
+  "v_mfma_f32_16x16x32_bf16 %[c12], %[q1], %[l2], %[c12]\n\t" \
+  "v_mfma_f32_16x16x32_bf16 %[c22], %[q2], %[l2], %[c22]\n\t" \
+  "global_load_lds_dwordx4 %[vt0], %[matb]\n\t" \
+  "v_add_u32 %[peb], %[stepb], %[peb]\n\t" \
+  "v_mfma_f32_16x16x32_bf16 %[c32], %[q3], %[l2], %[c32]\n\t" \
+  "v_mfma_f32_16x16x32_bf16 %[c42], %[q4], %[l2], %[c42]\n\t" \
+  "ds_read_b128 %[h5], %[x11] offset:10240\n\t" \
+  "v_mfma_f32_16x16x32_bf16 %[c52], %[q5], %[l2], %[c52]\n\t" \
+  "v_mfma_f32_16x16x32_bf16 %[c62], %[q6], %[l2], %[c62]\n\t" \
+  "v_mfma_f32_16x16x32_bf16 %[c72], %[q7], %[l2], %[c72]\n\t" \
+  "s_add_u32 m0, m0, 0x400\n\t" \
+  "v_min_u32 %[vt1], %[pob], %[vmaxb]\n\t" \
+  "v_mfma_f32_16x16x32_bf16 %[c03], %[q0], %[l3], %[c03]\n\t" \
+  "ds_read_b128 %[h6], %[x11] offset:12288\n\t" \
+  "v_mfma_f32_16x16x32_bf16 %[c13], %[q1], %[l3], %[c13]\n\t" \
+  "v_mfma_f32_16x16x32_bf16 %[c23], %[q2], %[l3], %[c23]\n\t" \
+  "global_load_lds_dwordx4 %[vt1], %[matb]\n\t" \
+  "v_add_u32 %[pob], %[stepb], %[pob]\n\t" \
+  "v_mfma_f32_16x16x32_bf16 %[c33], %[q3], %[l3], %[c33]\n\t" \
+  "v_mfma_f32_16x16x32_bf16 %[c43], %[q4], %[l3], %[c43]\n\t" \
+  "ds_read_b128 %[h7], %[x11] offset:14336\n\t" \
+  "v_mfma_f32_16x16x32_bf16 %[c53], %[q5], %[l3], %[c53]\n\t" \
+  "v_mfma_f32_16x16x32_bf16 %[c63], %[q6], %[l3], %[c63]\n\t" \
+  "v_mfma_f32_16x16x32_bf16 %[c73], %[q7], %[l3], %[c73]\n\t" \
+  "s_add_u32 m0, m0, 0x400\n\t" \
+  "v_min_u32 %[vt0], %[peb], %[vmaxb]\n\t" \
+  "v_mfma_f32_16x16x32_bf16 %[c00], %[q8], %[l4], %[c00]\n\t" \
+  "v_mfma_f32_16x16x32_bf16 %[c10], %[q9], %[l4], %[c10]\n\t" \
+  "v_mfma_f32_16x16x32_bf16 %[c20], %[q10], %[l4], %[c20]\n\t" \
+  "global_load_lds_dwordx4 %[vt0], %[matb]\n\t" \
+  "v_add_u32 %[peb], %[stepb], %[peb]\n\t" \
+  "v_mfma_f32_16x16x32_bf16 %[c30], %[q11], %[l4], %[c30]\n\t" \
+  "v_mfma_f32_16x16x32_bf16 %[c40], %[q12], %[l4], %[c40]\n\t" \
+  "v_mfma_f32_16x16x32_bf16 %[c50], %[q13], %[l4], %[c50]\n\t" \
+  "v_mfma_f32_16x16x32_bf16 %[c60], %[q14], %[l4], %[c60]\n\t" \
+  "v_mfma_f32_16x16x32_bf16 %[c70], %[q15], %[l4], %[c70]\n\t" \
+  "s_add_u32 m0, m0, 0x400\n\t" \
+  "v_min_u32 %[vt1], %[pob], %[vmaxb]\n\t" \
+  "v_mfma_f32_16x16x32_bf16 %[c01], %[q8], %[l5], %[c01]\n\t" \
+  "v_mfma_f32_16x16x32_bf16 %[c11], %[q9], %[l5], %[c11]\n\t" \
+  "v_mfma_f32_16x16x32_bf16 %[c21], %[q10], %[l5], %[c21]\n\t" \
+  "global_load_lds_dwordx4 %[vt1], %[matb]\n\t" \
+  "v_add_u32 %[pob], %[stepb], %[pob]\n\t" \
+  "v_mfma_f32_16x16x32_bf16 %[c31], %[q11], %[l5], %[c31]\n\t" \
+  "v_mfma_f32_16x16x32_bf16 %[c41], %[q12], %[l5], %[c41]\n\t" \
+  "v_mfma_f32_16x16x32_bf16 %[c51], %[q13], %[l5], %[c51]\n\t" \
+  "v_mfma_f32_16x16x32_bf16 %[c61], %[q14], %[l5], %[c61]\n\t" \
+  "v_mfma_f32_16x16x32_bf16 %[c71], %[q15], %[l5], %[c71]\n\t" \
+  "s_add_u32 m0, m0, 0x400\n\t" \
+  "v_min_u32 %[vt0], %[peb], %[vmaxb]\n\t" \
+  "v_mfma_f32_16x16x32_bf16 %[c02], %[q8], %[l6], %[c02]\n\t" \
+  "v_mfma_f32_16x16x32_bf16 %[c12], %[q9], %[l6], %[c12]\n\t" \
+  "v_mfma_f32_16x16x32_bf16 %[c22], %[q10], %[l6], %[c22]\n\t" \
+  "global_load_lds_dwordx4 %[vt0], %[matb]\n\t" \
+  "v_add_u32 %[peb], %[stepb], %[peb]\n\t" \
+  "v_mfma_f32_16x16x32_bf16 %[c32], %[q11], %[l6], %[c32]\n\t" \
+  "v_mfma_f32_16x16x32_bf16 %[c42], %[q12], %[l6], %[c42]\n\t" \
+  "v_mfma_f32_16x16x32_bf16 %[c52], %[q13], %[l6], %[c52]\n\t" \
+  "v_mfma_f32_16x16x32_bf16 %[c62], %[q14], %[l6], %[c62]\n\t" \
+  "v_mfma_f32_16x16x32_bf16 %[c72], %[q15], %[l6], %[c72]\n\t" \
+  "s_add_u32 m0, m0, 0x400\n\t" \
+  "v_min_u32 %[vt1], %[pob], %[vmaxb]\n\t" \
+  "v_mfma_f32_16x16x32_bf16 %[c03], %[q8], %[l7], %[c03]\n\t" \
+  "v_mfma_f32_16x16x32_bf16 %[c13], %[q9], %[l7], %[c13]\n\t" \
+  "v_mfma_f32_16x16x32_bf16 %[c23], %[q10], %[l7], %[c23]\n\t" \
+  "global_load_lds_dwordx4 %[vt1], %[matb]\n\t" \
+  "v_add_u32 %[pob], %[stepb], %[pob]\n\t" \
+  "v_mfma_f32_16x16x32_bf16 %[c33], %[q11], %[l7], %[c33]\n\t" \
+  "v_mfma_f32_16x16x32_bf16 %[c43], %[q12], %[l7], %[c43]\n\t" \
+  "v_mfma_f32_16x16x32_bf16 %[c53], %[q13], %[l7], %[c53]\n\t" \
+  "v_mfma_f32_16x16x32_bf16 %[c63], %[q14], %[l7], %[c63]\n\t" \
+  "v_mfma_f32_16x16x32_bf16 %[c73], %[q15], %[l7], %[c73]\n\t" \
+  "s_sub_u32 %[cc], %[cc], 1\n\t" \
+  "s_cmp_eq_u32 %[cc], 0\n\t" \
+  "s_cselect_b32 %[sadvb], %[tadvb], %[kadvb]\n\t" \
+  "s_cselect_b32 %[sadva], %[tadva], %[kadva]\n\t" \
+  "s_cselect_b32 %[cc], %[nkr], %[cc]\n\t" \
+  "v_add_u32 %[peb], %[sadvb], %[peb]\n\t" \
+  "v_add_u32 %[pob], %[sadvb], %[pob]\n\t" \
+  "s_waitcnt vmcnt(8) lgkmcnt(0)\n\t" \
+  "s_barrier\n\t" \
+  "s_mov_b32 m0, %[da1]\n\t" \
+  "v_min_u32 %[vt0], %[pea], %[vmaxa]\n\t" \
+  "v_mfma_f32_16x16x32_bf16 %[c04], %[q0], %[h0], %[c04]\n\t" \
+  "ds_read_b128 %[l0], %[x00] offset:0\n\t" \
+  "v_mfma_f32_16x16x32_bf16 %[c14], %[q1], %[h0], %[c14]\n\t" \
+  "ds_read_b128 %[l1], %[x00] offset:2048\n\t" \
+  "v_mfma_f32_16x16x32_bf16 %[c24], %[q2], %[h0], %[c24]\n\t" \
+  "global_load_lds_dwordx4 %[vt0], %[mata]\n\t" \
+  "v_add_u32 %[pea], %[stepa], %[pea]\n\t" \
+  "v_mfma_f32_16x16x32_bf16 %[c34], %[q3], %[h0], %[c34]\n\t" \
+  "v_mfma_f32_16x16x32_bf16 %[c44], %[q4], %[h0], %[c44]\n\t" \
+  "ds_read_b128 %[l2], %[x00] offset:4096\n\t" \
+  "v_mfma_f32_16x16x32_bf16 %[c54], %[q5], %[h0], %[c54]\n\t" \
+  "ds_read_b128 %[l3], %[x00] offset:6144\n\t" \
+  "v_mfma_f32_16x16x32_bf16 %[c64], %[q6], %[h0], %[c64]\n\t" \
+  "v_mfma_f32_16x16x32_bf16 %[c74], %[q7], %[h0], %[c74]\n\t" \
+  "s_add_u32 m0, m0, 0x400\n\t" \
+  "v_min_u32 %[vt1], %[poa], %[vmaxa]\n\t" \
+  "v_mfma_f32_16x16x32_bf16 %[c05], %[q0], %[h1], %[c05]\n\t" \
+  "ds_read_b128 %[p0], %[y00] offset:0\n\t" \
+  "v_mfma_f32_16x16x32_bf16 %[c15], %[q1], %[h1], %[c15]\n\t" \
+  "ds_read_b128 %[p1], %[y00] offset:2048\n\t" \
+  "v_mfma_f32_16x16x32_bf16 %[c25], %[q2], %[h1], %[c25]\n\t" \
+  "global_load_lds_dwordx4 %[vt1], %[mata]\n\t" \
+  "v_add_u32 %[poa], %[stepa], %[poa]\n\t" \
+  "v_mfma_f32_16x16x32_bf16 %[c35], %[q3], %[h1], %[c35]\n\t" \
+  "v_mfma_f32_16x16x32_bf16 %[c45], %[q4], %[h1], %[c45]\n\t" \
+  "ds_read_b128 %[p2], %[y00] offset:4096\n\t" \
+  "v_mfma_f32_16x16x32_bf16 %[c55], %[q5], %[h1], %[c55]\n\t" \
+  "ds_read_b128 %[p3], %[y00] offset:6144\n\t" \
+  "v_mfma_f32_16x16x32_bf16 %[c65], %[q6], %[h1], %[c65]\n\t" \
+  "v_mfma_f32_16x16x32_bf16 %[c75], %[q7], %[h1], %[c75]\n\t" \
+  "s_add_u32 m0, m0, 0x400\n\t" \
+  "v_min_u32 %[vt0], %[pea], %[vmaxa]\n\t" \
+  "v_mfma_f32_16x16x32_bf16 %[c06], %[q0], %[h2], %[c06]\n\t" \
+  "ds_read_b128 %[p4], %[y00] offset:8192\n\t" \
+  "v_mfma_f32_16x16x32_bf16 %[c16], %[q1], %[h2], %[c16]\n\t" \
+  "ds_read_b128 %[p5], %[y00] offset:10240\n\t" \
+  "v_mfma_f32_16x16x32_bf16 %[c26], %[q2], %[h2], %[c26]\n\t" \
+  "global_load_lds_dwordx4 %[vt0], %[mata]\n\t" \
+  "v_add_u32 %[pea], %[stepa], %[pea]\n\t" \
+  "v_mfma_f32_16x16x32_bf16 %[c36], %[q3], %[h2], %[c36]\n\t" \
+  "v_mfma_f32_16x16x32_bf16 %[c46], %[q4], %[h2], %[c46]\n\t" \
+  "ds_read_b128 %[p6], %[y00] offset:12288\n\t" \
+  "v_mfma_f32_16x16x32_bf16 %[c56], %[q5], %[h2], %[c56]\n\t" \
+  "ds_read_b128 %[p7], %[y00] offset:14336\n\t" \
+  "v_mfma_f32_16x16x32_bf16 %[c66], %[q6], %[h2], %[c66]\n\t" \
+  "v_mfma_f32_16x16x32_bf16 %[c76], %[q7], %[h2], %[c76]\n\t" \
+  "s_add_u32 m0, m0, 0x400\n\t" \
+  "v_min_u32 %[vt1], %[poa], %[vmaxa]\n\t" \
+  "v_mfma_f32_16x16x32_bf16 %[c07], %[q0], %[h3], %[c07]\n\t" \
+  "ds_read_b128 %[l4], %[x01] offset:0\n\t" \
+  "v_mfma_f32_16x16x32_bf16 %[c17], %[q1], %[h3], %[c17]\n\t" \
+  "ds_read_b128 %[l5], %[x01] offset:2048\n\t" \
+  "v_mfma_f32_16x16x32_bf16 %[c27], %[q2], %[h3], %[c27]\n\t" \
+  "global_load_lds_dwordx4 %[vt1], %[mata]\n\t" \
+  "v_add_u32 %[poa], %[stepa], %[poa]\n\t" \
+  "v_mfma_f32_16x16x32_bf16 %[c37], %[q3], %[h3], %[c37]\n\t" \
+  "v_mfma_f32_16x16x32_bf16 %[c47], %[q4], %[h3], %[c47]\n\t" \
+  "ds_read_b128 %[l6], %[x01] offset:4096\n\t" \
+  "v_mfma_f32_16x16x32_bf16 %[c57], %[q5], %[h3], %[c57]\n\t" \
+  "ds_read_b128 %[l7], %[x01] offset:6144\n\t" \
+  "v_mfma_f32_16x16x32_bf16 %[c67], %[q6], %[h3], %[c67]\n\t" \
+  "v_mfma_f32_16x16x32_bf16 %[c77], %[q7], %[h3], %[c77]\n\t" \
+  "s_add_u32 m0, m0, 0x400\n\t" \
+  "v_min_u32 %[vt0], %[pea], %[vmaxa]\n\t" \
+  "v_mfma_f32_16x16x32_bf16 %[c04], %[q8], %[h4], %[c04]\n\t" \
+  "ds_read_b128 %[p8], %[y01] offset:0\n\t" \
+  "v_mfma_f32_16x16x32_bf16 %[c14], %[q9], %[h4], %[c14]\n\t" \
+  "ds_read_b128 %[p9], %[y01] offset:2048\n\t" \
+  "v_mfma_f32_16x16x32_bf16 %[c24], %[q10], %[h4], %[c24]\n\t" \
+  "global_load_lds_dwordx4 %[vt0], %[mata]\n\t" \
+  "v_add_u32 %[pea], %[stepa], %[pea]\n\t" \
+  "v_mfma_f32_16x16x32_bf16 %[c34], %[q11], %[h4], %[c34]\n\t" \
+  "v_mfma_f32_16x16x32_bf16 %[c44], %[q12], %[h4], %[c44]\n\t" \
+  "ds_read_b128 %[p10], %[y01] offset:4096\n\t" \
+  "v_mfma_f32_16x16x32_bf16 %[c54], %[q13], %[h4], %[c54]\n\t" \
+  "ds_read_b128 %[p11], %[y01] offset:6144\n\t" \
+  "v_mfma_f32_16x16x32_bf16 %[c64], %[q14], %[h4], %[c64]\n\t" \
+  "v_mfma_f32_16x16x32_bf16 %[c74], %[q15], %[h4], %[c74]\n\t" \
+  "s_add_u32 m0, m0, 0x400\n\t" \
+  "v_min_u32 %[vt1], %[poa], %[vmaxa]\n\t" \
+  "v_mfma_f32_16x16x32_bf16 %[c05], %[q8], %[h5], %[c05]\n\t" \
+  "ds_read_b128 %[p12], %[y01] offset:8192\n\t" \
+  "v_mfma_f32_16x16x32_bf16 %[c15], %[q9], %[h5], %[c15]\n\t" \
+  "ds_read_b128 %[p13], %[y01] offset:10240\n\t" \
+  "v_mfma_f32_16x16x32_bf16 %[c25], %[q10], %[h5], %[c25]\n\t" \
+  "global_load_lds_dwordx4 %[vt1], %[mata]\n\t" \
+  "v_add_u32 %[poa], %[stepa], %[poa]\n\t" \
+  "v_mfma_f32_16x16x32_bf16 %[c35], %[q11], %[h5], %[c35]\n\t" \
+  "v_mfma_f32_16x16x32_bf16 %[c45], %[q12], %[h5], %[c45]\n\t" \
+  "ds_read_b128 %[p14], %[y01] offset:12288\n\t" \
+  "v_mfma_f32_16x16x32_bf16 %[c55], %[q13], %[h5], %[c55]\n\t" \
+  "ds_read_b128 %[p15], %[y01] offset:14336\n\t" \
+  "v_mfma_f32_16x16x32_bf16 %[c65], %[q14], %[h5], %[c65]\n\t" \
+  "v_mfma_f32_16x16x32_bf16 %[c75], %[q15], %[h5], %[c75]\n\t" \
+  "s_add_u32 m0, m0, 0x400\n\t" \
+  "v_min_u32 %[vt0], %[pea], %[vmaxa]\n\t" \
+  "v_mfma_f32_16x16x32_bf16 %[c06], %[q8], %[h6], %[c06]\n\t" \
+  "v_mfma_f32_16x16x32_bf16 %[c16], %[q9], %[h6], %[c16]\n\t" \
+  "v_mfma_f32_16x16x32_bf16 %[c26], %[q10], %[h6], %[c26]\n\t" \
+  "global_load_lds_dwordx4 %[vt0], %[mata]\n\t" \
+  "v_add_u32 %[pea], %[stepa], %[pea]\n\t" \
+  "v_mfma_f32_16x16x32_bf16 %[c36], %[q11], %[h6], %[c36]\n\t" \
+  "v_mfma_f32_16x16x32_bf16 %[c46], %[q12], %[h6], %[c46]\n\t" \
+  "v_mfma_f32_16x16x32_bf16 %[c56], %[q13], %[h6], %[c56]\n\t" \
+  "v_mfma_f32_16x16x32_bf16 %[c66], %[q14], %[h6], %[c66]\n\t" \
+  "v_mfma_f32_16x16x32_bf16 %[c76], %[q15], %[h6], %[c76]\n\t" \
+  "s_add_u32 m0, m0, 0x400\n\t" \
+  "v_min_u32 %[vt1], %[poa], %[vmaxa]\n\t" \
+  "v_mfma_f32_16x16x32_bf16 %[c07], %[q8], %[h7], %[c07]\n\t" \
+  "v_mfma_f32_16x16x32_bf16 %[c17], %[q9], %[h7], %[c17]\n\t" \
+  "v_mfma_f32_16x16x32_bf16 %[c27], %[q10], %[h7], %[c27]\n\t" \
+  "global_load_lds_dwordx4 %[vt1], %[mata]\n\t" \
+  "v_add_u32 %[poa], %[stepa], %[poa]\n\t" \
+  "v_mfma_f32_16x16x32_bf16 %[c37], %[q11], %[h7], %[c37]\n\t" \
+  "v_mfma_f32_16x16x32_bf16 %[c47], %[q12], %[h7], %[c47]\n\t" \
+  "v_mfma_f32_16x16x32_bf16 %[c57], %[q13], %[h7], %[c57]\n\t" \
+  "v_mfma_f32_16x16x32_bf16 %[c67], %[q14], %[h7], %[c67]\n\t" \
+  "v_mfma_f32_16x16x32_bf16 %[c77], %[q15], %[h7], %[c77]\n\t" \
+  "v_add_u32 %[pea], %[sadva], %[pea]\n\t" \
+  "v_add_u32 %[poa], %[sadva], %[poa]\n\t" \
+  "s_sub_u32 %[cnt], %[cnt], 1\n\t" \
+  "s_cmp_lg_u32 %[cnt], 0\n\t" \
+  "s_cbranch_scc1 1b\n\t" \
+  "s_waitcnt lgkmcnt(0)\n\t" \
+  "s_mov_b32 m0, %[sm]\n\t"
+
+#define W16_TILE_OUTS [c00] "+a"(acc[0][0]), [c01] "+a"(acc[0][1]), [c02] "+a"(acc[0][2]), [c03] "+a"(acc[0][3]), [c04] "+a"(acc[0][4]), [c05] "+a"(acc[0][5]), [c06] "+a"(acc[0][6]), [c07] "+a"(acc[0][7]), [c10] "+a"(acc[1][0]), [c11] "+a"(acc[1][1]), [c12] "+a"(acc[1][2]), [c13] "+a"(acc[1][3]), [c14] "+a"(acc[1][4]), [c15] "+a"(acc[1][5]), [c16] "+a"(acc[1][6]), [c17] "+a"(acc[1][7]), [c20] "+a"(acc[2][0]), [c21] "+a"(acc[2][1]), [c22] "+a"(acc[2][2]), [c23] "+a"(acc[2][3]), [c24] "+a"(acc[2][4]), [c25] "+a"(acc[2][5]), [c26] "+a"(acc[2][6]), [c27] "+a"(acc[2][7]), [c30] "+a"(acc[3][0]), [c31] "+a"(acc[3][1]), [c32] "+a"(acc[3][2]), [c33] "+a"(acc[3][3]), [c34] "+a"(acc[3][4]), [c35] "+a"(acc[3][5]), [c36] "+a"(acc[3][6]), [c37] "+a"(acc[3][7]), [c40] "+a"(acc[4][0]), [c41] "+a"(acc[4][1]), [c42] "+a"(acc[4][2]), [c43] "+a"(acc[4][3]), [c44] "+a"(acc[4][4]), [c45] "+a"(acc[4][5]), [c46] "+a"(acc[4][6]), [c47] "+a"(acc[4][7]), [c50] "+a"(acc[5][0]), [c51] "+a"(acc[5][1]), [c52] "+a"(acc[5][2]), [c53] "+a"(acc[5][3]), [c54] "+a"(acc[5][4]), [c55] "+a"(acc[5][5]), [c56] "+a"(acc[5][6]), [c57] "+a"(acc[5][7]), [c60] "+a"(acc[6][0]), [c61] "+a"(acc[6][1]), [c62] "+a"(acc[6][2]), [c63] "+a"(acc[6][3]), [c64] "+a"(acc[6][4]), [c65] "+a"(acc[6][5]), [c66] "+a"(acc[6][6]), [c67] "+a"(acc[6][7]), [c70] "+a"(acc[7][0]), [c71] "+a"(acc[7][1]), [c72] "+a"(acc[7][2]), [c73] "+a"(acc[7][3]), [c74] "+a"(acc[7][4]), [c75] "+a"(acc[7][5]), [c76] "+a"(acc[7][6]), [c77] "+a"(acc[7][7]), [l0] "+v"(fl[0]), [l1] "+v"(fl[1]), [l2] "+v"(fl[2]), [l3] "+v"(fl[3]), [l4] "+v"(fl[4]), [l5] "+v"(fl[5]), [l6] "+v"(fl[6]), [l7] "+v"(fl[7]), [p0] "+v"(fp[0]), [p1] "+v"(fp[1]), [p2] "+v"(fp[2]), [p3] "+v"(fp[3]), [p4] "+v"(fp[4]), [p5] "+v"(fp[5]), [p6] "+v"(fp[6]), [p7] "+v"(fp[7]), [p8] "+v"(fp[8]), [p9] "+v"(fp[9]), [p10] "+v"(fp[10]), [p11] "+v"(fp[11]), [p12] "+v"(fp[12]), [p13] "+v"(fp[13]), [p14] "+v"(fp[14]), [p15] "+v"(fp[15]), [h0] "=&v"(fh[0]), [h1] "=&v"(fh[1]), [h2] "=&v"(fh[2]), [h3] "=&v"(fh[3]), [h4] "=&v"(fh[4]), [h5] "=&v"(fh[5]), [h6] "=&v"(fh[6]), [h7] "=&v"(fh[7]), [q0] "=&v"(fq[0]), [q1] "=&v"(fq[1]), [q2] "=&v"(fq[2]), [q3] "=&v"(fq[3]), [q4] "=&v"(fq[4]), [q5] "=&v"(fq[5]), [q6] "=&v"(fq[6]), [q7] "=&v"(fq[7]), [q8] "=&v"(fq[8]), [q9] "=&v"(fq[9]), [q10] "=&v"(fq[10]), [q11] "=&v"(fq[11]), [q12] "=&v"(fq[12]), [q13] "=&v"(fq[13]), [q14] "=&v"(fq[14]), [q15] "=&v"(fq[15])
+#define W16_TILE_ADDRS [x00] "v"(adX[0][0]), [x01] "v"(adX[0][1]), [x10] "v"(adX[1][0]), [x11] "v"(adX[1][1]), [y00] "v"(adY[0][0]), [y01] "v"(adY[0][1]), [y10] "v"(adY[1][0]), [y11] "v"(adY[1][1])
```

Result: no change. 757.0, median of 6 (+0.4%).
